# evfro/polara

Measured on AMD Instinct MI355X. Metric: users scored/sec + SVD build time, ML-20M rank-50 PureSVD, higher is better.
Workload: dtype bf16x3

## Files before the change

### include/polara_hip.h

```cpp
#ifndef POLARA_HIP_H
#define POLARA_HIP_H

#include <stdint.h>

#ifdef __cplusplus
extern "C" {
#endif

#define PK_OK 0
#define PK_E_INVALID (-1)
#define PK_E_LAUNCH (-2)
#define PK_E_UNSUPPORTED (-3)
#define PK_E_NOCONV (-4)

#define PK_VAL_F32 0
#define PK_VAL_F64 1

const char *pk_last_error(void);
int pk_version(void);
int pk_set_option(const char *name, int32_t value, int32_t unset);
int pk_copy_to_host_async(void *stream, void *dst_host, const void *src_dev, int64_t bytes);
int pk_device_info(int device, char *name, int name_len, int *cu_count, int64_t *hbm_bytes);
int pk_warm_up(void);

// ... 73 lines not shown
int pk_orth_check_f64(void *stream, int32_t l, const double *G_dev, int64_t ldg, int32_t *info_dev, int32_t n_info,
                      double *flags_dev);
int pk_eigh_psd_f64(void *stream, int32_t n, double *S_dev, int64_t lds_, double *evecs_dev, int64_t ldv,
                    double *evals_dev, int32_t max_sweeps, double tol, int32_t *info_dev);
int pk_eigh_psd_rounds_f64(void *stream, int32_t n, double *S_dev, int64_t lds_, double *evecs_dev, int64_t ldv,
                           double *evals_dev, int32_t max_sweeps, double tol, int32_t *info_dev);
int pk_eigh_top_supported(int32_t n, int32_t r);
int64_t pk_eigh_top_work_bytes(int32_t n);
int pk_eigh_top_f64(void *stream, int32_t n, const double *S_dev, int64_t lds_, int32_t r, double *evecs_dev, int64_t ldv,
                    double *evals_dev, void *work_dev, int32_t *info_dev);
int64_t pk_chol_work_bytes(int32_t n);
int pk_chol_rinv_f64(void *stream, int32_t n, const double *G_dev, int64_t ldg, double shift_rel, double *Rinv_dev,
                     int64_t ldr, void *work_dev, int32_t *info_dev);
int pk_chol_rinv_scaled_f64(void *stream, int32_t n, const double *G_dev, int64_t ldg, double shift_rel, double *Rinv_dev,
                     int64_t ldr, void *work_dev, int32_t *info_dev);
int pk_axpbypcz_f64(void *stream, int64_t n_elems, double alpha, const double *Z_dev, double beta,
                    const double *Y_dev, double gamma, const double *X_dev, double *out_dev);
int32_t pk_resid_blocks(int64_t n);
int pk_resid_colnorm2_f64(void *stream, int64_t n, int32_t l, const double *Z_dev, int64_t ldz,
                          const double *X_dev, int64_t ldx, const double *theta_dev, double *partial_dev);
int pk_dgemm_small_f64(void *stream, int transA, int transB, int32_t M, int32_t N, int32_t K,
                       const double *A_dev, int64_t lda, const double *B_dev, int64_t ldb,
                       double *C_dev, int64_t ldc);
int pk_scale_cols_f64(void *stream, int64_t n, int32_t l, double *X_dev, int64_t ldx, const double *s_dev);

int64_t pk_pack_elems(int64_t n, int32_t K);
int32_t pk_pack_kq(int32_t K);
int pk_pack_frag_f32(void *stream, int64_t n, int32_t K, const double *src_dev, int64_t ld, float *dst_dev);
int32_t pk_candidate_capacity(int32_t topk);
int64_t pk_score_state_bytes(int64_t n_users, int32_t splits);
int32_t pk_score_splits(int64_t n_users, int32_t KC);
int pk_seen_tiles_build(void *stream, int64_t n_users, const int64_t *seen_ptr_dev, const int32_t *seen_idx_dev,
                        int32_t rows_sorted ,
                        int64_t max_row_len ,
                        uint64_t *tiles_dev, int32_t *ntiles_dev);
int32_t pk_seen_tiles_max_unsorted_row(void);
int pk_score_candidates_f32(void *stream, int64_t n_users, int64_t n_items, int32_t K,
                            const float *Vp_dev, const float *Ep_dev,
                            const int64_t *seen_ptr_dev, const uint64_t *seen_tiles_dev,
                            const int32_t *seen_ntiles_dev ,
                            int32_t KC, int32_t splits ,
                            float *cand_score_dev, int32_t *cand_idx_dev ,
                            void *state_dev ,
                            int32_t tiles_per_chunk ,
                            const float *user_bound_dev ,
                            const float *tile_bound_dev ,
                            const uint32_t *seen_dense_dev, const int32_t *seen_skip_dev,
                            int32_t dense_tiles );
int pk_sweep_takes_rows(void);
int pk_score_candidates_rows_f32(void *stream, int64_t n_users, int64_t n_items, int32_t K, const float *Vp_dev,
                                 const double *E_dev, int64_t lde, const double *extra_dev, int64_t extra_ld,
                                 double extra_scale, const int64_t *seen_ptr_dev, const uint64_t *seen_tiles_dev,
                                 const int32_t *seen_ntiles_dev, int32_t KC, int32_t splits, float *cand_score_dev,
                                 int32_t *cand_idx_dev, void *state_dev, int32_t tiles_per_chunk ,
                                 const float *tile_bound_dev , const uint32_t *seen_dense_dev,
                                 const int32_t *seen_skip_dev, int32_t dense_tiles);
int pk_score_two_phase_plan(int64_t n_users, int64_t n_items, int32_t KC, int32_t *head_tiles, int32_t *splits);
int pk_score_two_phase_f32(void *stream, int64_t n_users, int64_t n_items, int32_t K,
                           const float *Vp_dev, const float *Ep_dev,
                           const int64_t *seen_ptr_dev, const uint64_t *seen_tiles_dev, const int32_t *seen_ntiles_dev,
                           int32_t KC, int32_t head_tiles, int32_t splits ,
                           float *work_score_dev, int32_t *work_idx_dev, float *cand_score_dev, int32_t *cand_idx_dev,
                           void *state_dev, int32_t tiles_per_chunk ,
                           const float *user_bound_dev, const float *tile_bound_dev ,
                           const uint32_t *seen_dense_dev, const int32_t *seen_skip_dev, int32_t dense_tiles);
int pk_score_two_phase_rows_f32(void *stream, int64_t n_users, int64_t n_items, int32_t K, const float *Vp_dev,
                                const double *E_dev, int64_t lde, const double *extra_dev, int64_t extra_ld,
                                double extra_scale, const int64_t *seen_ptr_dev, const uint64_t *seen_tiles_dev,
                                const int32_t *seen_ntiles_dev, int32_t KC, int32_t head_tiles, int32_t splits,
                                float *work_score_dev, int32_t *work_idx_dev, float *cand_score_dev, int32_t *cand_idx_dev,
                                void *state_dev, int32_t tiles_per_chunk, const float *tile_bound_dev,
                                const uint32_t *seen_dense_dev, const int32_t *seen_skip_dev, int32_t dense_tiles);
int64_t pk_seen_dense_bytes(int64_t n_users, int32_t dense_tiles);
int pk_seen_dense_build(void *stream, int64_t n_users, const int64_t *seen_ptr_dev, const uint64_t *seen_tiles_dev,
                        const int32_t *seen_ntiles_dev, int32_t dense_tiles, uint32_t *dense_dev, int32_t *skip_dev);
int32_t pk_score_chunk_launches(int64_t n_items, int32_t K, int32_t splits, int32_t tiles_per_chunk, int32_t pruned);
int pk_row_norm_bound_f32(void *stream, int64_t n, int32_t K, const double *src_dev, int64_t ld, float *out_dev);
int pk_v32_image_f32(void *stream, int64_t n, int32_t K, int32_t ld32, const double *V_dev, int64_t ldv, const float *bound_dev,
                     float *out_dev, uint32_t *stat_dev);
int pk_pack_frag_bound_f32(void *stream, int64_t n, int32_t K, const double *src_dev, int64_t ld, float *dst_dev,
                           float *bound_dev, const double *extra_dev, int64_t extra_ld, double extra_scale);
int pk_tile_norm_bound_f32(void *stream, int64_t n_items, int32_t K, const double *V_dev, int64_t ld,
                           float *work_dev, float *out_dev);
int pk_rescore_topk_f64(void *stream, int64_t n_users, int64_t n_items, int32_t K,
                        const double *V_dev, int64_t ldv, const double *E_dev, int64_t lde,
                        const int64_t *seen_ptr_dev, int32_t KC, int32_t splits,
                        const float *cand_score_dev, const int32_t *cand_idx_dev, int32_t topk,
                        double v_row_norm_max,
                        int64_t *out_idx_dev, double *out_score_dev , int32_t *flags_dev);
int pk_rescore_topk_rows_f64(void *stream, int64_t n_rows, const int32_t *rows_dev,
                             const int32_t *n_rows_dev ,
                             int64_t n_users, int64_t n_items,
                             int32_t K, const double *V_dev, int64_t ldv,
                             const float *V32_dev , int64_t ldv32,
                             const double *E_dev, int64_t lde,
                             const double *e_err_dev, int64_t e_err_ld ,
                             int32_t e_exact ,
                             const int64_t *seen_ptr_dev, int32_t KC, int32_t splits,
                             const float *cand_score_dev, const int32_t *cand_idx_dev, int32_t topk,
                             double v_row_norm_max,
                             int64_t *out_idx_dev, double *out_score_dev , int32_t *flags_dev);
int pk_rescore_topk_rows_list_f64(void *stream, int64_t n_rows, const int32_t *rows_dev,
                             const int32_t *n_rows_dev ,
                             int64_t n_users, int64_t n_items,
                             int32_t K, const double *V_dev, int64_t ldv,
                             const float *V32_dev , int64_t ldv32,
                             const double *E_dev, int64_t lde,
                             const double *e_err_dev, int64_t e_err_ld ,
                             int32_t e_exact ,
                             const int64_t *seen_ptr_dev, int32_t KC, int32_t splits,
                             const float *cand_score_dev, const int32_t *cand_idx_dev, int32_t topk,
                             double v_row_norm_max,
                             int64_t *out_idx_dev, double *out_score_dev , int32_t *flags_dev,
                             int32_t *flagged_list_dev, int32_t *flagged_count_dev, int32_t flagged_offset);
int pk_rescore_topk_rows_norms_f64(void *stream, int64_t n_rows, const int32_t *rows_dev,
                             const int32_t *n_rows_dev, int64_t n_users, int64_t n_items,
                             int32_t K, const double *V_dev, int64_t ldv,
                             const float *V32_dev, int64_t ldv32,
                             const double *E_dev, int64_t lde,
                             const double *e_err_dev, int64_t e_err_ld, int32_t e_exact,
                             const int64_t *seen_ptr_dev, int32_t KC, int32_t splits,
                             const float *cand_score_dev, const int32_t *cand_idx_dev, int32_t topk,
                             double v_row_norm_max,
                             int64_t *out_idx_dev, double *out_score_dev, int32_t *flags_dev,
                             int32_t *flagged_list_dev, int32_t *flagged_count_dev, int32_t flagged_offset,
                             const float *item_norm_dev);
int pk_rescore_topk_rows_perm_f64(void *stream, int64_t n_rows, const int32_t *rows_dev,
                             const int32_t *n_rows_dev, int64_t n_users, int64_t n_items,
                             int32_t K, const double *V_dev, int64_t ldv,
                             const float *V32_dev, int64_t ldv32,
                             const double *E_dev, int64_t lde,
                             const double *e_err_dev, int64_t e_err_ld, int32_t e_exact,
                             const int64_t *seen_ptr_dev, int32_t KC, int32_t splits,
                             const float *cand_score_dev, const int32_t *cand_idx_dev, int32_t topk,
                             double v_row_norm_max,
                             int64_t *out_idx_dev, double *out_score_dev, int32_t *flags_dev,
                             int32_t *flagged_list_dev, int32_t *flagged_count_dev, int32_t flagged_offset,
                             const float *item_norm_dev, const int64_t *out_perm_dev);
int pk_zero_i32(void *stream, int32_t *p_dev, int32_t n);
int pk_flag_compact(void *stream, int64_t n, const int32_t *flags_dev, int32_t mask, int32_t *list_dev,
                    int32_t *count_dev);
int pk_fold_rows_f64(void *stream, int64_t cap, const int32_t *list_dev, const int32_t *count_dev, int64_t row_offset,
                     const int64_t *indptr_dev, const int32_t *indices_dev, const void *vals_dev, int val_kind,
                     const double *V_dev, int64_t ldv, int32_t K, double *E_dev, int64_t lde);

int pk_spmm_csr_flagged_f64(void *stream, int64_t n_tasks, const int32_t *task_row_dev, const int64_t *task_begin_dev,
                            const int64_t *task_end_dev, const int32_t *task_slot_dev, int64_t n_long,
                            const int32_t *long_row_dev, const int32_t *long_slot_begin_dev,
                            const int32_t *long_slot_end_dev, const int32_t *indices_dev, const void *vals_dev,
                            int val_kind, const double *X_dev, int64_t ldx, int32_t nc, double *out_dev, int64_t ldo,
                            double *partial_dev, int64_t x_rows, const int32_t *row_flags_dev, int32_t flag_mask);

int pk_spmm_csr_rows_list_f64(void *stream, int64_t cap, const int32_t *list_dev, const int32_t *count_dev, int64_t row_offset,
                              const int64_t *row_first_task_dev, const int32_t *task_row_dev, const int64_t *task_begin_dev,
                              const int64_t *task_end_dev, const int32_t *task_slot_dev, int64_t n_long,
                              const int32_t *long_row_dev, const int32_t *long_slot_begin_dev, const int32_t *long_slot_end_dev,
                              const int32_t *indices_dev, const void *vals_dev, int val_kind, const double *X_dev, int64_t ldx,
                              int32_t nc, double *out_dev, int64_t ldo, double *partial_dev, int64_t x_rows,
                              const int32_t *row_flags_dev, int32_t flag_mask);

int32_t pk_q20_lanes(int32_t K);
double pk_q20_kappa(int32_t K);
int64_t pk_q20_image_bytes(int64_t n, int32_t K);
int pk_q20_encode_f64(void *stream, int64_t n, int32_t K, const double *V_dev, int64_t ldv, void *img_dev,
                      double *tab_dev, void *work_dev, int32_t *info_dev);
int pk_q20_decode_f64(void *stream, int64_t n, int32_t K, const void *img_dev, const double *tab_dev, double *out_dev,
// ... 167 lines not shown
```

### polara_amd/_lib.py

```python
import ctypes as C
import os

_HERE = os.path.dirname(os.path.abspath(__file__))
LIB_PATH = os.environ.get('POLARA_HIP_LIB') or os.path.join(_HERE, 'libpolarahip.so')

PK_VAL_F32, PK_VAL_F64 = 0, 1

_vp, _i32, _i64, _f64 = C.c_void_p, C.c_int32, C.c_int64, C.c_double

PROTOTYPES = {
    'pk_last_error': (C.c_char_p, []),
    'pk_version': (C.c_int, []),
    'pk_warm_up': (C.c_int, []),
    'pk_device_info': (C.c_int, [C.c_int, C.c_char_p, C.c_int, C.POINTER(C.c_int), C.POINTER(_i64)]),
    'pk_spmm_csr_f64': (C.c_int, [_vp, _i64, _vp, _vp, _vp, _vp, _i64, _vp, _vp, _vp, _vp, _vp, C.c_int,
                                  _vp, _i64, _i32, _vp, _i64, _vp]),
    'pk_spmm_csr_x': (C.c_int, [_vp, _i64, _vp, _vp, _vp, _vp, _i64, _vp, _vp, _vp, _vp, _vp, C.c_int,
                                _vp, C.c_int, _i64, _i32, _vp, _i64, _vp]),
    'pk_spmm_csr_ex': (C.c_int, [_vp, _i64, _vp, _vp, _vp, _vp, _i64, _vp, _vp, _vp, _vp, _vp, C.c_int,
                                 _vp, C.c_int, _i64, _i32, _vp, _i64, _vp, _i64, _i32, _i64]),
    'pk_scan_work_bytes': (_i64, [_i64]),
    'pk_exclusive_scan_i32': (C.c_int, [_vp, _i64, _vp, _vp, _vp]),
    'pk_radix_work_bytes': (_i64, [_i64]),
    'pk_radix_sort_pairs': (C.c_int, [_vp, _i64, _i32, _vp, _vp, _vp, _vp, _i32, _vp, C.POINTER(_i32)]),
    'pk_coo_to_csr_work_bytes': (_i64, [_i64]),
    'pk_coo_to_csr': (C.c_int, [_vp, _i64, _vp, _vp, _i64, _vp, C.c_int, _i64, _i64, _vp, _vp, _vp, _vp, _vp, _vp]),
    'pk_csr_transpose_work_bytes': (_i64, [_i64]),
    'pk_csr_transpose': (C.c_int, [_vp, _i64, _i64, _i64, _vp, _vp, _vp, C.c_int, _i64, _vp, _vp, _vp, _vp]),
    'pk_csr_relabel_work_bytes': (_i64, [_i64]),
    'pk_csr_relabel_sorted': (C.c_int, [_vp, _i64, _i64, _i64, _vp, _vp, _vp, C.c_int, _vp, _vp, _vp, _vp]),
    'pk_csr_rows_by_length_work_bytes': (_i64, [_i64]),
    'pk_csr_rows_by_length': (C.c_int, [_vp, _i64, _i64, _vp, _vp, _vp, C.c_int, _vp, _vp, _vp, _vp, _vp]),
    'pk_count_i32': (C.c_int, [_vp, _i64, _vp, _i64, _vp]),
    'pk_csr_scale_f64': (C.c_int, [_vp, _i64, _vp, _vp, _vp, C.c_int, _vp, _vp, _vp]),
    'pk_row_plan_work_bytes': (_i64, [_i64]),
    'pk_row_plan_count': (C.c_int, [_vp, _i64, _vp, _i32, _vp, _vp]),
    'pk_row_plan_fill': (C.c_int, [_vp, _i64, _vp, _vp, _vp, _vp, _vp, _vp, _vp, _vp, _vp, _vp, _vp]),
    'pk_gram_work_bytes': (_i64, [_i64, _i32, _i32]),
    'pk_gram_f64': (C.c_int, [_vp, _i64, _i32, _i32, _vp, _i64, _vp, _i64, _vp, _i64, _vp]),
    'pk_tsmm_f64': (C.c_int, [_vp, _i64, _i32, _i32, _vp, _i64, _vp, _i64, _vp, _i64]),
    'pk_tsmm_sub_f64': (C.c_int, [_vp, _i64, _i32, _i32, _vp, _i64, _vp, _i64, _vp, _i64, _vp, _i64]),
    'pk_tsmm_axpby_f64': (C.c_int, [_vp, _i64, _i32, _i32, _vp, _i64, _vp, _i64, _f64, _f64, _vp, _i64, _f64, _vp, _i64, _vp, _i64]),
    'pk_orth_check_f64': (C.c_int, [_vp, _i32, _vp, _i64, _vp, _i32, _vp]),
    'pk_eigh_psd_f64': (C.c_int, [_vp, _i32, _vp, _i64, _vp, _i64, _vp, _i32, _f64, _vp]),
    'pk_eigh_psd_rounds_f64': (C.c_int, [_vp, _i32, _vp, _i64, _vp, _i64, _vp, _i32, _f64, _vp]),
    'pk_eigh_top_supported': (C.c_int, [_i32, _i32]),
    'pk_eigh_top_work_bytes': (_i64, [_i32]),
    'pk_eigh_top_f64': (C.c_int, [_vp, _i32, _vp, _i64, _i32, _vp, _i64, _vp, _vp, _vp]),
    'pk_chol_work_bytes': (_i64, [_i32]),
    'pk_chol_rinv_f64': (C.c_int, [_vp, _i32, _vp, _i64, _f64, _vp, _i64, _vp, _vp]),
    'pk_chol_rinv_scaled_f64': (C.c_int, [_vp, _i32, _vp, _i64, _f64, _vp, _i64, _vp, _vp]),
    'pk_axpbypcz_f64': (C.c_int, [_vp, _i64, _f64, _vp, _f64, _vp, _f64, _vp, _vp]),
    'pk_resid_blocks': (_i32, [_i64]),
    'pk_resid_colnorm2_f64': (C.c_int, [_vp, _i64, _i32, _vp, _i64, _vp, _i64, _vp, _vp]),
    'pk_dgemm_small_f64': (C.c_int, [_vp, C.c_int, C.c_int, _i32, _i32, _i32, _vp, _i64, _vp, _i64, _vp, _i64]),
    'pk_scale_cols_f64': (C.c_int, [_vp, _i64, _i32, _vp, _i64, _vp]),
    'pk_pack_elems': (_i64, [_i64, _i32]),
    'pk_pack_kq': (_i32, [_i32]),
    'pk_pack_frag_f32': (C.c_int, [_vp, _i64, _i32, _vp, _i64, _vp]),
    'pk_candidate_capacity': (_i32, [_i32]),
    'pk_score_state_bytes': (_i64, [_i64, _i32]),
    'pk_score_splits': (_i32, [_i64, _i32]),
    'pk_seen_tiles_build': (C.c_int, [_vp, _i64, _vp, _vp, _i32, _i64, _vp, _vp]),
    'pk_seen_tiles_max_unsorted_row': (_i32, []),
    'pk_score_candidates_f32': (C.c_int, [_vp, _i64, _i64, _i32, _vp, _vp, _vp, _vp, _vp, _i32, _i32, _vp, _vp, _vp,
                                          _i32, _vp, _vp, _vp, _vp, _i32]),
    'pk_score_candidates_rows_f32': (C.c_int, [_vp, _i64, _i64, _i32, _vp, _vp, _i64, _vp, _i64, _f64, _vp, _vp, _vp, _i32, _i32,
                                               _vp, _vp, _vp, _i32, _vp, _vp, _vp, _i32]),
    'pk_score_two_phase_rows_f32': (C.c_int, [_vp, _i64, _i64, _i32, _vp, _vp, _i64, _vp, _i64, _f64, _vp, _vp, _vp, _i32, _i32, _i32,
                                              _vp, _vp, _vp, _vp, _vp, _i32, _vp, _vp, _vp, _i32]),
    'pk_score_two_phase_plan': (C.c_int, [_i64, _i64, _i32, _vp, _vp]),
    'pk_score_two_phase_f32': (C.c_int, [_vp, _i64, _i64, _i32, _vp, _vp, _vp, _vp, _vp, _i32, _i32, _i32, _vp, _vp, _vp, _vp, _vp,
                                         _i32, _vp, _vp, _vp, _vp, _i32]),
    'pk_seen_dense_bytes': (_i64, [_i64, _i32]),
    'pk_seen_dense_build': (C.c_int, [_vp, _i64, _vp, _vp, _vp, _i32, _vp, _vp]),
    'pk_score_chunk_launches': (_i32, [_i64, _i32, _i32, _i32, _i32]),
    'pk_pack_frag_bound_f32': (C.c_int, [_vp, _i64, _i32, _vp, _i64, _vp, _vp, _vp, _i64, _f64]),
    'pk_row_norm_bound_f32': (C.c_int, [_vp, _i64, _i32, _vp, _i64, _vp]),
    'pk_tile_norm_bound_f32': (C.c_int, [_vp, _i64, _i32, _vp, _i64, _vp, _vp]),
    'pk_rescore_topk_f64': (C.c_int, [_vp, _i64, _i64, _i32, _vp, _i64, _vp, _i64, _vp, _i32, _i32, _vp, _vp,
                                      _i32, _f64, _vp, _vp, _vp]),
    'pk_flag_compact': (C.c_int, [_vp, _i64, _vp, _i32, _vp, _vp]),
    'pk_fold_rows_f64': (C.c_int, [_vp, _i64, _vp, _vp, _i64, _vp, _vp, _vp, C.c_int, _vp, _i64, _i32, _vp, _i64]),
    'pk_spmm_csr_flagged_f64': (C.c_int, [_vp, _i64, _vp, _vp, _vp, _vp, _i64, _vp, _vp, _vp, _vp, _vp, C.c_int, _vp, _i64, _i32,
                                          _vp, _i64, _vp, _i64, _vp, _i32]),
    'pk_spmm_csr_rows_list_f64': (C.c_int, [_vp, _i64, _vp, _vp, _i64, _vp, _vp, _vp, _vp, _vp, _i64, _vp, _vp, _vp, _vp, _vp, C.c_int,
                                            _vp, _i64, _i32, _vp, _i64, _vp, _i64, _vp, _i32]),
    'pk_q20_lanes': (_i32, [_i32]),
    'pk_q20_kappa': (_f64, [_i32]),
    'pk_q20_image_bytes': (_i64, [_i64, _i32]),
    'pk_q20_encode_f64': (C.c_int, [_vp, _i64, _i32, _vp, _i64, _vp, _vp, _vp, _vp]),
    'pk_q20_decode_f64': (C.c_int, [_vp, _i64, _i32, _vp, _vp, _vp, _i64]),
    'pk_fold_q20': (C.c_int, [_vp, _i64, _vp, _vp, _vp, _vp, _i64, _vp, _vp, _vp, _vp, _vp, C.c_int, _vp, _vp, _i64, _i32, _i32,
                              _vp, _i64, _vp]),
    'pk_fold_q20_zero': (C.c_int, [_vp, _i64, _vp, _vp, _vp, _vp, _i64, _vp, _vp, _vp, _vp, _vp, C.c_int, _vp, _vp, _i64, _i32, _i32,
                                   _vp, _i64, _vp, _vp, _i32]),
    'pk_rescore_topk_rows_f64': (C.c_int, [_vp, _i64, _vp, _vp, _i64, _i64, _i32, _vp, _i64, _vp, _i64, _vp, _i64, _vp, _i64, _i32, _vp, _i32, _i32,
                                           _vp, _vp, _i32, _f64, _vp, _vp, _vp]),
    'pk_rescore_topk_rows_list_f64': (C.c_int, [_vp, _i64, _vp, _vp, _i64, _i64, _i32, _vp, _i64, _vp, _i64, _vp, _i64, _vp, _i64, _i32, _vp, _i32, _i32,
                                           _vp, _vp, _i32, _f64, _vp, _vp, _vp, _vp, _vp, _i32]),
    'pk_rescore_topk_rows_norms_f64': (C.c_int, [_vp, _i64, _vp, _vp, _i64, _i64, _i32, _vp, _i64, _vp, _i64, _vp, _i64, _vp, _i64, _i32, _vp, _i32, _i32,
                                           _vp, _vp, _i32, _f64, _vp, _vp, _vp, _vp, _vp, _i32, _vp]),
    'pk_rescore_topk_rows_perm_f64': (C.c_int, [_vp, _i64, _vp, _vp, _i64, _i64, _i32, _vp, _i64, _vp, _i64, _vp, _i64, _vp, _i64, _i32, _vp, _i32, _i32,
                                           _vp, _vp, _i32, _f64, _vp, _vp, _vp, _vp, _vp, _i32, _vp, _vp]),
    'pk_zero_i32': (C.c_int, [_vp, _vp, _i32]),
    'pk_scatter_rows_i64': (C.c_int, [_vp, _i64, _i32, _vp, _vp, _vp]),
    'pk_map_ids_i64': (C.c_int, [_vp, _i64, _vp, _vp, _i64, _vp]),
    'pk_exact_work_bytes': (_i64, [_i32, _i64]),
    'pk_score_exact_rows_f64': (C.c_int, [_vp, _i32, _vp, _i64, _i32, _vp, _i64, _vp, _i64, _vp, _vp, _i32,
                                          _vp, _vp, _vp]),
    'pk_score_exact_list_f64': (C.c_int, [_vp, _i32, _vp, _vp, _i64, _i32, _vp, _i64, _vp, _i64, _vp, _vp, _i32,
                                          _vp, _vp, _vp]),
    'pk_score_exact_list_perm_f64': (C.c_int, [_vp, _i32, _vp, _vp, _i64, _i32, _vp, _i64, _vp, _i64, _vp, _vp, _i32,
                                               _vp, _vp, _vp, _vp]),
    'pk_exact_work_init': (C.c_int, [_vp, _vp, _i32, _i64]),
    'pk_eval_ranks': (C.c_int, [_vp, _i64, _vp, _i32, _vp, _vp, _vp]),
    'pk_eval_cols': (_i32, []),
    'pk_eval_user_metrics': (C.c_int, [_vp, _i64, _i32, _vp, _i64, _vp, _vp, _vp, _vp, _f64, _f64, _i32, _vp]),
    'pk_eval_reduce_work_bytes': (_i64, [_i64]),
    'pk_eval_reduce': (C.c_int, [_vp, _i64, _vp, _vp, _vp]),
    'pk_unique_count_i64': (C.c_int, [_vp, _i64, _vp, _i64, _vp, _vp]),
    'pk_dense_scores_f64': (C.c_int, [_vp, _i32, _i64, _i32, _vp, _i64, _vp, _i64, _vp, _i64]),
    'pk_topk_rows_f64': (C.c_int, [_vp, _i64, _i64, _vp, _i64, _i32, _vp]),
    'pk_i2i_max_topk': (_i32, []),
    'pk_i2i_window': (_i32, []),
    'pk_i2i_build_window': (_i32, []),
    'pk_i2i_ld': (_i64, [_i64]),
    'pk_i2i_chunk_users': (_i64, [_i64, _i64, _i32]),
    'pk_i2i_topk_work_bytes': (_i64, [_i64, _i64, _i32]),
    'pk_i2i_build_f64': (C.c_int, [_vp, _i64, _i64, _vp, _vp, _vp, C.c_int, _vp, _vp, _vp, _vp, _i64]),
    'pk_i2i_image_f32': (C.c_int, [_vp, _i64, _vp, _vp, _vp]),
    'pk_i2i_topk': (C.c_int, [_vp, _i64, _i64, _vp, _vp, _vp, C.c_int, _vp, C.c_int, _i64, _i32, _i32, _i32, _vp, _vp, _vp]),
    'pk_popular_order_work_bytes': (_i64, [_i64]),
    'pk_popular_order': (C.c_int, [_vp, _i64, _vp, _vp, _vp]),
    'pk_popular_topk': (C.c_int, [_vp, _i64, _i64, _vp, _vp, _vp, _i32, _i32, _vp]),
    'pk_hybrid_ld': (_i64, [_i64]),
    'pk_hybrid_max_nc': (_i32, []),
    'pk_trmm_work_bytes': (_i64, [_i64, _i32]),
    'pk_hybrid_densify_f64': (C.c_int, [_vp, _i64, _vp, _vp, _vp, _vp, _f64, _vp, _i64]),
    'pk_chol_f64': (C.c_int, [_vp, _i64, _vp, _i64, _vp]),
    'pk_trmm_f64': (C.c_int, [_vp, _i32, _i64, _i32, _vp, _i64, _vp, _i64, _vp, _i64, _vp]),
    'pk_trsm_f64': (C.c_int, [_vp, _i64, _i32, _vp, _i64, _vp, _i64]),
    'pk_lce_fused_max_rank': (_i32, []),
    'pk_lce_update_f64': (C.c_int, [_vp, _i64, _i32, _vp, _i64, _vp, _i64, _vp, _i64, _f64, _vp, _i64, _f64, _f64, _f64, _vp]),
    'pk_lce_update_ew_f64': (C.c_int, [_vp, _i64, _i32, _vp, _i64, _vp, _i64, _vp, _i64, _f64, _f64, _vp]),
    'pk_lce_dot_blocks': (_i32, [_i64]),
    'pk_lce_dots_work_bytes': (_i64, []),
    'pk_lce_dots_f64': (C.c_int, [_vp, _i32, _vp, _vp, _vp, _vp, _vp, _vp, _vp, _vp, _f64, _vp, _vp]),
    'pk_clamp_min_f64': (C.c_int, [_vp, _i64, _i32, _vp, _i64, _f64]),
    'pk_ctx_create': (C.c_int, [_i32, C.POINTER(_vp)]),
    'pk_ctx_destroy': (None, [_vp]),
    'pk_ctx_error': (C.c_char_p, [_vp]),
    'pk_mat_from_csr': (C.c_int, [_vp, _i64, _i64, _i64, _vp, _vp, _vp, _i32, C.POINTER(_vp)]),
# ... 75 lines not shown
```

### polara_amd/csrc/api.cpp

```cpp
#include "pk_common.h"
#include <string.h>

static thread_local char g_err[512] = "";

void pk_set_error(const char *fmt, ...) {
    va_list ap;
    va_start(ap, fmt);
    vsnprintf(g_err, sizeof(g_err), fmt, ap);
    va_end(ap);
}

extern "C" const char *pk_last_error(void) { return g_err; }

#include <atomic>
namespace {
struct Option { const char *name; std::atomic<int> value; std::atomic<bool> set; };
Option g_options[] = {{"score_boot_tiles", {0}, {false}}, {"score_head_tiles", {0}, {false}}, {"score_phase2_splits", {0}, {false}}};
}
int pk_option(const char *name, int dflt) {
    for (auto &o : g_options)
        if (!strcmp(o.name, name)) return o.set.load() ? o.value.load() : dflt;
    return dflt;
}
extern "C" int pk_set_option(const char *name, int32_t value, int32_t unset) {
    if (name)
        for (auto &o : g_options)
            if (!strcmp(o.name, name)) {
                o.value.store(value);
                o.set.store(!unset);
                return PK_OK;
            }
    pk_set_error("pk_set_option: unknown option '%s'", name ? name : "(null)");
    return PK_E_INVALID;
}
extern "C" int pk_version(void) { return 100; }

extern "C" int pk_copy_to_host_async(void *stream, void *dst_host, const void *src_dev, int64_t bytes) {
    if (bytes < 0 || (bytes > 0 && (!dst_host || !src_dev))) {
        pk_set_error("pk_copy_to_host_async: bad arguments");
        return PK_E_INVALID;
    }
    if (bytes == 0) return PK_OK;
    const hipError_t e = hipMemcpyAsync(dst_host, src_dev, (size_t)bytes, hipMemcpyDeviceToHost, static_cast<hipStream_t>(stream));
    if (e != hipSuccess) {
        pk_set_error("pk_copy_to_host_async: %s", hipGetErrorString(e));
        return PK_E_LAUNCH;
    }
    return PK_OK;
}

extern "C" int pk_device_info(int device, char *name, int name_len, int *cu_count, int64_t *hbm_bytes) {
    int n = 0;
    hipError_t e = hipGetDeviceCount(&n);
    if (e != hipSuccess || n <= 0) {
        pk_set_error("pk_device_info: no HIP device visible (%s)", hipGetErrorString(e));
        return PK_E_LAUNCH;
    }
    if (device < 0 || device >= n) {
        pk_set_error("pk_device_info: device %d out of range [0,%d)", device, n);
        return PK_E_INVALID;
    }
    hipDeviceProp_t prop;
    e = hipGetDeviceProperties(&prop, device);
    if (e != hipSuccess) {
        pk_set_error("pk_device_info: %s", hipGetErrorString(e));
        return PK_E_LAUNCH;
    }
    if (name && name_len > 0) {
        strncpy(name, prop.gcnArchName, name_len - 1);
        name[name_len - 1] = 0;
    }
    if (cu_count) *cu_count = prop.multiProcessorCount;
    if (hbm_bytes) *hbm_bytes = (int64_t)prop.totalGlobalMem;
    return n;
}

hipError_t pk_tu_load_dense();
hipError_t pk_tu_load_driver();
hipError_t pk_tu_load_eigh();
hipError_t pk_tu_load_eigh_top();
hipError_t pk_tu_load_evalmetrics();
hipError_t pk_tu_load_hybrid();
hipError_t pk_tu_load_i2i();
hipError_t pk_tu_load_foldq();
hipError_t pk_tu_load_ingest();
hipError_t pk_tu_load_lce();
hipError_t pk_tu_load_rescore();
hipError_t pk_tu_load_score();
hipError_t pk_tu_load_spmm();
hipError_t pk_tu_load_ttm();

extern "C" int pk_warm_up(void) {
    hipError_t (*const loaders[])() = {pk_tu_load_dense, pk_tu_load_driver, pk_tu_load_eigh, pk_tu_load_eigh_top, pk_tu_load_evalmetrics, pk_tu_load_foldq, pk_tu_load_hybrid, pk_tu_load_i2i, pk_tu_load_ingest, pk_tu_load_lce, pk_tu_load_rescore, pk_tu_load_score, pk_tu_load_spmm, pk_tu_load_ttm};
    for (auto f : loaders) {
        const hipError_t e = f();
        if (e != hipSuccess) {
            pk_set_error("pk_warm_up: %s", hipGetErrorString(e));
            return PK_E_LAUNCH;
        }
    }
// ... 3 lines not shown
```

### polara_amd/csrc/driver.hip

```cpp
#include "pk_common.h"
#include <algorithm>
#include <cmath>
#include <cstdarg>
#include <cstring>
#include <map>
#include <memory>
#include <mutex>
#include <numeric>
#include <random>
#include <string>
#include <type_traits>
#include <vector>

namespace model {
constexpr double kDenseF64Flops = 20e12;
constexpr double kLanczosStepFixedS = 0.3e-3;
constexpr double kNestedSolveS = 1.5e-3;
constexpr double kXgmiBusBps = 100e9;
constexpr double kCollectiveStepS = 5e-6;
}

struct DevPool {
    std::multimap<size_t, void *> free_blocks;
    void *get(size_t &bytes) {
// ... 1682 lines not shown
    HIPCK(hipMemcpy2DAsync(Z_dev, (size_t)ldz * 8, Z.p(), (size_t)nc * 8, (size_t)nc * 8, (size_t)n, hipMemcpyDeviceToDevice, ctx->stream));
    return PK_OK;
}

__global__ void v32_image_stat_kernel(int64_t n, int K, int ld32, const double *__restrict__ V, int64_t ldv, const float *__restrict__ bound,
                                      float *__restrict__ out, uint32_t *__restrict__ stat) {
    const int64_t i = (int64_t)blockIdx.x * blockDim.x + threadIdx.x;
    if (i >= n * ld32) return;
    const int64_t r = i / ld32;
    const int c = (int)(i - r * ld32);
    float v = 0.0f;
    if (c < K) {
        const double d = V[r * ldv + c];
        v = (float)d;
        if (!(fabs(d) <= 1.7976931348623157e308)) atomicOr(&stat[1], 1u);
    } else if (c == K) {
        v = bound[r];
        if (!(v >= 0.0f && v <= 3.4028234e38f)) atomicOr(&stat[1], 1u); else atomicMax(&stat[0], __float_as_uint(v));
    }
    out[i] = v;
}

extern "C" int pk_v32_image_f32(void *stream, int64_t n, int32_t K, int32_t ld32, const double *V_dev, int64_t ldv, const float *bound_dev,
                                float *out_dev, uint32_t *stat_dev) {
    PK_REQUIRE(n >= 0 && K >= 1 && ld32 > K && ldv >= K && V_dev && bound_dev && out_dev && stat_dev, "pk_v32_image_f32: bad arguments");
    hipStream_t st = pk_stream(stream);
    (void)hipMemsetAsync(stat_dev, 0, 8, st);
    if (n > 0)
        hipLaunchKernelGGL(v32_image_stat_kernel, dim3((unsigned)(((size_t)n * ld32 + 255) / 256)), dim3(256), 0, st, n, K, ld32, V_dev, ldv, bound_dev,
                           out_dev, stat_dev);
    PK_CHECK_LAUNCH("v32_image_stat_kernel");
    return PK_OK;
}

extern "C" int pk_sym_eig_topk_f64(pk_ctx *ctx, void *stream, int32_t n, const double *T_dev, int64_t ldt, int32_t k, int32_t l,
                                   const double *X0_dev, int64_t ldx0, int32_t x0_rows, double tol, int32_t max_outer, uint64_t seed,
                                   double *basis_out_dev, int64_t ldb, double *lam_out_host, double *res_out_host,
                                   int32_t *counts_out, const double *lam0_host, double r0_rel) {
    if (!ctx) return PK_E_INVALID;
    std::lock_guard<std::mutex> lock(ctx->mu);
    PoolScope pool_scope(ctx);
    (void)hipSetDevice(ctx->device);
    if (n < 1 || k < 1 || l < k || l > n || l > 1024 || !T_dev || ldt < n || !basis_out_dev || ldb < l || !lam_out_host || !res_out_host ||
        !counts_out || (X0_dev && (x0_rows < 1 || x0_rows > n || ldx0 < l)))
        return fail(ctx, PK_E_INVALID, "pk_sym_eig_topk_f64: bad arguments (n=%d, k=%d, l=%d)", n, k, l);
    if (tol <= 0) tol = 1e-13;
    if (max_outer <= 0) max_outer = 200;
    hipStream_t st = stream ? pk_stream(stream) : ctx->stream;
    Solver S{ctx, st, Dev()};
    DMat T(n, n), X(n, l);
    if (!T.ok() || !X.ok()) return fail(ctx, PK_E_LAUNCH, "out of device memory (pk_sym_eig_topk_f64)");
    HIPCK(hipMemcpy2DAsync(T.p(), (size_t)n * 8, T_dev, (size_t)ldt * 8, (size_t)n * 8, (size_t)n, hipMemcpyDeviceToDevice, st));
    if (X0_dev) {
        HIPCK(hipMemsetAsync(X.p(), 0, (size_t)n * l * 8, st));
        HIPCK(hipMemcpy2DAsync(X.p(), (size_t)l * 8, X0_dev, (size_t)ldx0 * 8, (size_t)l * 8, (size_t)x0_rows, hipMemcpyDeviceToDevice, st));
    } else {
        hipLaunchKernelGGL(unit_block_kernel, dim3((unsigned)(((int64_t)n * l + 255) / 256)), dim3(256), 0, st, (int64_t)n, l, X.p());
    }
    DenseOp dop{ctx, S, T};
    SubspaceOut so;
    CK(dense_topk(ctx, S, dop, k, std::move(X), tol, max_outer, seed, X0_dev ? lam0_host : nullptr, r0_rel, so, X0_dev == nullptr));
    const int w = std::min<int>(l, so.basis.l);
    HIPCK(hipMemcpy2DAsync(basis_out_dev, (size_t)ldb * 8, so.basis.p(), (size_t)so.basis.l * 8, (size_t)w * 8, (size_t)n,
                           hipMemcpyDeviceToDevice, st));
    HIPCK(hipStreamSynchronize(st));
    for (int j = 0; j < l; ++j) lam_out_host[j] = j < (int)so.lam_all.size() ? so.lam_all[(size_t)j] : 0.0;
    for (int j = 0; j < l; ++j) res_out_host[j] = j < (int)so.res_act.size() ? so.res_act[(size_t)j] : 0.0;
    counts_out[0] = so.n_lock;
    counts_out[1] = w - so.n_lock;
    counts_out[2] = so.converged ? 1 : 0;
    counts_out[3] = so.outer;
    counts_out[4] = dop.products;
    return PK_OK;
}

struct pk_serving {
    int64_t n_items = 0, n_users = 0;
    int K = 0, ld32 = 0, Kx_full = 0;
    double vmax = 0.0;
    bool nonneg = true, have_tiles = false, have_v32 = false, fused = false;
    Dev inv64;
    DMat V;
    Csr Ts;
    Dev Vp, tile_bound, V32, tiles, ntiles, dense, skip;
    Dev vnorm, q20_raw, q20_tab;
    char *q20_img = nullptr;
    int dense_tiles = 0;
    Dev exact_work;
};

namespace {

int serving_build(pk_ctx *ctx, pk_serving *sv, int64_t n_items, int32_t K, const double *V_host, pk_mat *T) {
    hipStream_t st = ctx->stream;
    const int64_t n_users = T->A.n_rows;
    Solver S{ctx, st, Dev()};
    sv->n_items = n_items; sv->n_users = n_users; sv->K = K; sv->nonneg = T->nonneg; sv->fused = K <= 256;
    std::vector<double> norm((size_t)n_items, 0.0);
    for (int j = 0; j < K; ++j)
        for (int64_t i = 0; i < n_items; ++i) { const double v = V_host[(size_t)j * n_items + i]; norm[(size_t)i] += v * v; }
    double vmax = 0.0;
    for (auto &v : norm) { v = std::sqrt(v); vmax = std::max(vmax, v); }
    if (!std::isfinite(vmax) || (vmax != 0.0 && !(vmax > 1e-30 && vmax < 1e30)))
        return fail(ctx, PK_E_INVALID, "pk_score_topk: item factors with max row norm %g are outside the fp32 range of the candidate sweep", vmax);
    sv->vmax = vmax;
    std::vector<int32_t> inv((size_t)n_items), rank_of((size_t)n_items);
    std::iota(inv.begin(), inv.end(), 0);
    std::stable_sort(inv.begin(), inv.end(), [&](int32_t a, int32_t b) { return norm[(size_t)a] > norm[(size_t)b]; });
    for (int64_t i = 0; i < n_items; ++i) rank_of[(size_t)inv[(size_t)i]] = (int32_t)i;
    {
        std::vector<int64_t> inv_l(inv.begin(), inv.end());
        if (!sv->inv64.alloc((size_t)n_items * 8)) return fail(ctx, PK_E_LAUNCH, "out of device memory (item ids)");
        CK(S.upload(inv_l.data(), sv->inv64.p, (size_t)n_items * 8));
    }
    std::vector<double> vr((size_t)n_items * K);
    for (int64_t i = 0; i < n_items; ++i)
        for (int j = 0; j < K; ++j) vr[(size_t)i * K + j] = V_host[(size_t)j * n_items + inv[(size_t)i]];
    sv->V = DMat(n_items, K);
    DMat &V = sv->V;
    if (!V.ok()) return fail(ctx, PK_E_LAUNCH, "out of device memory (factors)");
    CK(S.upload(vr.data(), V.p(), vr.size() * 8));
    Csr &Ts = sv->Ts;
    Ts.n_rows = n_users; Ts.n_cols = n_items; Ts.nnz = T->A.nnz; Ts.val_kind = T->A.val_kind;
    const size_t ve = Ts.val_kind == PK_VAL_F32 ? 4 : 8, n1 = (size_t)std::max<int64_t>(Ts.nnz, 1);
    {
        Dev cmap((size_t)n_items * 4), work((size_t)pk_csr_relabel_work_bytes(Ts.nnz));
        if (!cmap.p || !work.p || !Ts.indptr.alloc((size_t)(n_users + 1) * 8) || !Ts.indices.alloc(n1 * 4) || !Ts.values.alloc(n1 * ve))
            return fail(ctx, PK_E_LAUNCH, "out of device memory (test matrix)");
        CK(S.upload(rank_of.data(), cmap.p, (size_t)n_items * 4));
        HIPCK(hipMemcpyAsync(Ts.indptr.p, T->A.indptr.p, (size_t)(n_users + 1) * 8, hipMemcpyDeviceToDevice, st));
        CK(pk_csr_relabel_sorted(st, n_users, n_items, Ts.nnz, T->A.indptr.as<int64_t>(), T->A.indices.as<int32_t>(), T->A.values.p,
                                 Ts.val_kind, cmap.as<int32_t>(), Ts.indices.as<int32_t>(), Ts.values.p, work.p));
        HIPCK(hipStreamSynchronize(st));
    }
    CK(build_plan(ctx, Ts));
    if (!sv->fused) return PK_OK;
    Dev tb_work((size_t)n_items * 4), rowb((size_t)n_items * 4);
    if (!sv->Vp.alloc((size_t)pk_pack_elems(n_items, K) * 4) || !sv->tile_bound.alloc((size_t)((n_items + 31) / 32) * 4) || !tb_work.p || !rowb.p)
        return fail(ctx, PK_E_LAUNCH, "out of device memory (factor images)");
    CK(pk_pack_frag_f32(st, n_items, K, V.p(), K, sv->Vp.as<float>()));
    CK(pk_tile_norm_bound_f32(st, n_items, K, V.p(), K, tb_work.as<float>(), sv->tile_bound.as<float>()));
    sv->Kx_full = ((K + 1 + 3) / 4) * 4;
    sv->ld32 = sv->Kx_full > 16 ? ((sv->Kx_full + 31) / 32) * 32 : (sv->Kx_full <= 4 ? 4 : sv->Kx_full <= 8 ? 8 : 16);
    if (sv->Kx_full <= 256 && sv->nonneg) {
        if (!sv->V32.alloc((size_t)n_items * sv->ld32 * 4)) return fail(ctx, PK_E_LAUNCH, "out of device memory (fp32 image)");
        CK(pk_row_norm_bound_f32(st, n_items, K, V.p(), K, rowb.as<float>()));
        hipLaunchKernelGGL(v32_image_kernel, dim3((unsigned)(((size_t)n_items * sv->ld32 + 255) / 256)), dim3(256), 0, st, n_items, K, sv->ld32,
                           V.p(), rowb.as<float>(), sv->V32.as<float>());
        sv->have_v32 = true;
        if (!sv->vnorm.alloc((size_t)n_items * 4)) return fail(ctx, PK_E_LAUNCH, "out of device memory (item norms)");
        HIPCK(hipMemcpyAsync(sv->vnorm.p, rowb.p, (size_t)n_items * 4, hipMemcpyDeviceToDevice, st));
        const int64_t qbytes = pk_q20_image_bytes(n_items, K);
        if (qbytes > 0 && n_items < (1 << 24) && qbytes < ((int64_t)1 << 32)) {
            Dev qwork(768), qinfo(4);
            if (!sv->q20_raw.alloc((size_t)qbytes + 128) || !sv->q20_tab.alloc(96 * 8) || !qwork.p || !qinfo.p)
                return fail(ctx, PK_E_LAUNCH, "out of device memory (packed image)");
            char *img = static_cast<char *>(sv->q20_raw.p);
            img += (128 - (reinterpret_cast<uintptr_t>(img) & 127)) & 127;
            CK(pk_q20_encode_f64(st, n_items, K, V.p(), K, img, sv->q20_tab.as<double>(), qwork.p, qinfo.as<int32_t>()));
            int32_t info = 0;
            CK(S.to_host(qinfo.p, &info, 4));
            if (info == 0) sv->q20_img = img;
        }
    }
    HIPCK(hipStreamSynchronize(st));
    return PK_OK;
}

int serving_score(pk_ctx *ctx, pk_serving *sv, int32_t topk, int32_t filter_seen, int64_t *out_idx, double *out_scores) {
    hipStream_t st = ctx->stream;
    const int64_t n_items = sv->n_items, n_users = sv->n_users;
    const int K = sv->K;
    if (!out_idx || topk < 1) return fail(ctx, PK_E_INVALID, "pk_score_topk: bad arguments");
    if (topk > n_items) return fail(ctx, PK_E_INVALID, "kth(=%lld) out of bounds (%lld)", (long long)(n_items - topk), (long long)n_items);
    Solver S{ctx, st, Dev()};
    DMat &V = sv->V;
    Csr &Ts = sv->Ts;
    const double vmax = sv->vmax;
    const size_t n1 = (size_t)std::max<int64_t>(Ts.nnz, 1);
    const Range all{0, Ts.plan.n_tasks, 0, Ts.plan.n_long};
    const int64_t *seen_ptr = filter_seen ? Ts.indptr.as<int64_t>() : nullptr;
    const int32_t *seen_idx = filter_seen ? Ts.indices.as<int32_t>() : nullptr;
    Dev out_i((size_t)n_users * topk * 8), out_s((size_t)n_users * topk * 8), flags((size_t)n_users * 4), lst((size_t)std::max<int64_t>(n_users, 1) * 4), cnt(4);
    Dev lst2((size_t)std::max<int64_t>(n_users, 1) * 4), cnt2(8);
    if (!out_i.p || !out_s.p || !flags.p || !lst.p || !cnt.p || !lst2.p || !cnt2.p) return fail(ctx, PK_E_LAUNCH, "out of device memory (outputs)");
    const int KC = sv->fused ? pk_candidate_capacity(topk) : 0;
    const int n_wg = 128;
    Dev &exact_work = sv->exact_work;
    if (!exact_work.p) {
        if (!exact_work.alloc((size_t)pk_exact_work_bytes(n_wg, n_items))) return fail(ctx, PK_E_LAUNCH, "out of device memory (exact rows)");
        CK(pk_exact_work_init(st, exact_work.p, n_wg, n_items));
    }
    if (KC == 0) {
        DMat E(n_users, K);
        if (!E.ok()) return fail(ctx, PK_E_LAUNCH, "out of device memory (E)");
        CK(spmm(ctx, Ts, V.p(), PK_VAL_F64, K, K, E.p(), K, all));
        hipLaunchKernelGGL(iota_i32_kernel, dim3((unsigned)((n_users + 255) / 256)), dim3(256), 0, st, n_users, lst.as<int32_t>(), cnt.as<int32_t>());
        CK(pk_score_exact_list_f64(st, n_wg, lst.as<int32_t>(), cnt.as<int32_t>(), n_items, K, V.p(), K, E.p(), K, seen_ptr, seen_idx, topk,
                                   out_i.as<int64_t>(), out_s.as<double>(), exact_work.p));
        HIPCK(hipStreamSynchronize(st));
    } else {
        const bool approx = !out_scores && sv->have_v32;
        const int Kx = approx ? sv->Kx_full : K, ld32 = sv->ld32;
        DMat Ex(n_users, Kx);
        if (!Ex.ok()) return fail(ctx, PK_E_LAUNCH, "out of device memory (E)");
        bool counters_zeroed = false;
        if (approx && sv->q20_img && topk <= 20) {
            Plan &P = Ts.plan;
            const size_t need = (size_t)P.n_slots * Kx * 8;
            if (need > P.partial.bytes && !P.partial.alloc(need)) return fail(ctx, PK_E_LAUNCH, "out of device memory (fold-in partials)");
            CK(pk_fold_q20_zero(st, all.nt, P.task_row.as<int32_t>() + all.t0, P.task_begin.as<int64_t>() + all.t0,
                                P.task_end.as<int64_t>() + all.t0, P.task_slot.as<int32_t>() + all.t0, all.nl,
                                P.long_row.as<int32_t>() + all.l0, P.long_sb.as<int32_t>() + all.l0, P.long_se.as<int32_t>() + all.l0,
                                Ts.indices.as<int32_t>(), Ts.values.p, Ts.val_kind, sv->q20_img, sv->q20_tab.as<double>(), n_items, K, Kx,
                                Ex.p(), Kx, P.partial.as<double>(), cnt2.as<int32_t>(), 2));
            counters_zeroed = true;
        } else if (approx) CK(spmm(ctx, Ts, sv->V32.p, PK_VAL_F32, ld32, Kx, Ex.p(), Kx, all));
        else CK(spmm(ctx, Ts, V.p(), PK_VAL_F64, K, K, Ex.p(), Kx, all));
        const double *w = approx ? Ex.p() + K : nullptr;
        const bool from_rows = (Kx % 2 == 0) && (((uintptr_t)Ex.p()) % 16 == 0);
        Dev Ep, ub;
        if (!from_rows) {
            if (!Ep.alloc((size_t)pk_pack_elems(n_users, K) * 4) || !ub.alloc((size_t)n_users * 4))
                return fail(ctx, PK_E_LAUNCH, "out of device memory (E fragments)");
            CK(pk_pack_frag_bound_f32(st, n_users, K, Ex.p(), Kx, Ep.as<float>(), ub.as<float>(), w, approx ? Kx : 0, 1.2e-7));
        }
        if (filter_seen && !sv->have_tiles) {
            if (!sv->tiles.alloc(n1 * 8) || !sv->ntiles.alloc((size_t)n_users * 4)) return fail(ctx, PK_E_LAUNCH, "out of device memory (seen tiles)");
            CK(pk_seen_tiles_build(st, n_users, Ts.indptr.as<int64_t>(), Ts.indices.as<int32_t>(), 1, 0, sv->tiles.as<uint64_t>(), sv->ntiles.as<int32_t>()));
            sv->have_tiles = true;
            const int64_t n_tiles_all = (n_items + 31) / 32, groups = (n_users + 31) / 32;
            int dt = (int)std::min<int64_t>(n_tiles_all, 256);
            while (dt > 32 && groups * dt * 128 > ((int64_t)512 << 20)) dt /= 2;
            if (n_tiles_all <= 32 * (int64_t)dt && sv->dense.alloc((size_t)pk_seen_dense_bytes(n_users, dt)) &&
                sv->skip.alloc((size_t)n_users * 4)) {
                CK(pk_seen_dense_build(st, n_users, Ts.indptr.as<int64_t>(), sv->tiles.as<uint64_t>(), sv->ntiles.as<int32_t>(), dt,
                                       sv->dense.as<uint32_t>(), sv->skip.as<int32_t>()));
                sv->dense_tiles = dt;
            }
        }
        const uint64_t *tiles = filter_seen ? sv->tiles.as<uint64_t>() : nullptr;
        const int32_t *ntiles = filter_seen ? sv->ntiles.as<int32_t>() : nullptr;
        int splits = ((n_users + 31) / 32) * 8 > 2048 ? 1 : pk_score_splits(n_users, KC);
        const int64_t n_pad = ((n_users + 31) / 32) * 32;
        int32_t head_tiles = 0, splits2 = 0;
        CK(pk_score_two_phase_plan(n_users, n_items, KC, &head_tiles, &splits2));
        const int slots = head_tiles ? splits2 + 1 : splits;
        Dev state((size_t)pk_score_state_bytes(n_users, slots)), cs((size_t)slots * n_pad * KC * 4), ci((size_t)slots * n_pad * KC * 4);
        Dev ms(head_tiles ? (size_t)n_pad * KC * 4 : 0), mi(head_tiles ? (size_t)n_pad * KC * 4 : 0);
        if (!state.p || !cs.p || !ci.p || (head_tiles && (!ms.p || !mi.p))) return fail(ctx, PK_E_LAUNCH, "out of device memory (candidates)");
        const uint32_t *dense_p = (filter_seen && sv->dense_tiles) ? sv->dense.as<uint32_t>() : nullptr;
        const int32_t *skip_p = (filter_seen && sv->dense_tiles) ? sv->skip.as<int32_t>() : nullptr;
        if (head_tiles) {
            if (from_rows)
                CK(pk_score_two_phase_rows_f32(st, n_users, n_items, K, sv->Vp.as<float>(), Ex.p(), Kx, w, approx ? Kx : 0, 1.2e-7, seen_ptr,
                                               tiles, ntiles, KC, head_tiles, splits2, cs.as<float>(), ci.as<int32_t>(), ms.as<float>(),
                                               mi.as<int32_t>(), state.p, 0, sv->tile_bound.as<float>(), dense_p, skip_p,
                                               filter_seen ? sv->dense_tiles : 0));
            else
                CK(pk_score_two_phase_f32(st, n_users, n_items, K, sv->Vp.as<float>(), Ep.as<float>(), seen_ptr, tiles, ntiles, KC, head_tiles,
                                          splits2, cs.as<float>(), ci.as<int32_t>(), ms.as<float>(), mi.as<int32_t>(), state.p, 0, ub.as<float>(),
                                          sv->tile_bound.as<float>(), dense_p, skip_p, filter_seen ? sv->dense_tiles : 0));
            std::swap(cs, ms);
            std::swap(ci, mi);
            splits = 1;
        } else if (from_rows) {
            CK(pk_score_candidates_rows_f32(st, n_users, n_items, K, sv->Vp.as<float>(), Ex.p(), Kx, w, approx ? Kx : 0, 1.2e-7, seen_ptr,
                                            tiles, ntiles, KC, splits, cs.as<float>(), ci.as<int32_t>(), state.p, 0,
                                            sv->tile_bound.as<float>(), dense_p, skip_p, filter_seen ? sv->dense_tiles : 0));
        } else {
            CK(pk_score_candidates_f32(st, n_users, n_items, K, sv->Vp.as<float>(), Ep.as<float>(), seen_ptr, tiles, ntiles,
                                       KC, splits, cs.as<float>(), ci.as<int32_t>(), state.p, 0, ub.as<float>(), sv->tile_bound.as<float>(),
                                       dense_p, skip_p, filter_seen ? sv->dense_tiles : 0));
        }
        if (!counters_zeroed) CK(pk_zero_i32(st, cnt2.as<int32_t>(), 2));
        int32_t *c_refold = cnt2.as<int32_t>(), *c_final = cnt2.as<int32_t>() + 1;
        CK(pk_rescore_topk_rows_norms_f64(st, n_users, nullptr, nullptr, n_users, n_items, K, V.p(), K, approx ? sv->V32.as<float>() : nullptr, approx ? ld32 : 0,
                                          Ex.p(), Kx, w, approx ? Kx : 0, 0, seen_ptr, KC, splits, cs.as<float>(), ci.as<int32_t>(), topk, vmax,
                                          out_i.as<int64_t>(), out_s.as<double>(), flags.as<int32_t>(),
                                          approx ? lst.as<int32_t>() : lst2.as<int32_t>(), approx ? c_refold : c_final, 0,
                                          approx ? sv->vnorm.as<float>() : nullptr));
        if (approx) {
            if ((K & 1) == 0 && K >= 2) {
                Plan &P = Ts.plan;
                const size_t need = (size_t)P.n_slots * K * 8;
                if (need > P.partial.bytes && !P.partial.alloc(need)) return fail(ctx, PK_E_LAUNCH, "out of device memory (re-fold partials)");
                CK(pk_spmm_csr_rows_list_f64(st, n_users, lst.as<int32_t>(), c_refold, 0, P.row_first_task.as<int64_t>(), P.task_row.as<int32_t>(),
                                             P.task_begin.as<int64_t>(), P.task_end.as<int64_t>(), P.task_slot.as<int32_t>(), all.nl,
                                             P.long_row.as<int32_t>() + all.l0, P.long_sb.as<int32_t>() + all.l0, P.long_se.as<int32_t>() + all.l0,
                                             Ts.indices.as<int32_t>(), Ts.values.p, Ts.val_kind, V.p(), K, K, Ex.p(), Kx, P.partial.as<double>(),
                                             n_items, flags.as<int32_t>(), 7));
            } else
            CK(pk_fold_rows_f64(st, n_users, lst.as<int32_t>(), c_refold, 0, Ts.indptr.as<int64_t>(), Ts.indices.as<int32_t>(), Ts.values.p,
                                Ts.val_kind, V.p(), K, K, Ex.p(), Kx));
            CK(pk_rescore_topk_rows_list_f64(st, n_users, lst.as<int32_t>(), c_refold, n_users, n_items, K, V.p(), K, nullptr, 0, Ex.p(), Kx, w, Kx,
                                             1, seen_ptr, KC, splits, cs.as<float>(), ci.as<int32_t>(), topk, vmax, out_i.as<int64_t>(), out_s.as<double>(),
                                             flags.as<int32_t>(), lst2.as<int32_t>(), c_final, 0));
        }
        CK(pk_score_exact_list_f64(st, n_wg, lst2.as<int32_t>(), c_final, n_items, K, V.p(), K, Ex.p(), Kx, seen_ptr, seen_idx, topk,
                                   out_i.as<int64_t>(), out_s.as<double>(), exact_work.p));
        HIPCK(hipStreamSynchronize(st));
    }
    Dev ext((size_t)n_users * topk * 8);
    if (!ext.p) return fail(ctx, PK_E_LAUNCH, "out of device memory (outputs)");
    CK(pk_map_ids_i64(st, n_users * (int64_t)topk, out_i.as<int64_t>(), sv->inv64.as<int64_t>(), n_items, ext.as<int64_t>()));
    CK(S.to_host(ext.p, out_idx, (size_t)n_users * topk * 8));
    if (out_scores) CK(S.to_host(out_s.p, out_scores, (size_t)n_users * topk * 8));
    return PK_OK;
}

}

extern "C" int pk_serving_create(pk_ctx *ctx, int64_t n_items, int32_t K, const double *V_host, pk_mat *T, pk_serving **out) {
    if (!ctx || !T || !out) return PK_E_INVALID;
    std::lock_guard<std::mutex> lock(ctx->mu);
    PoolScope pool_scope(ctx);
    (void)hipSetDevice(ctx->device);
    *out = nullptr;
    if (n_items != T->A.n_cols) return fail(ctx, PK_E_INVALID, "pk_score_topk: test matrix and item factors disagree on the number of items");
    if (K < 1 || K > 8192 || !V_host) return fail(ctx, PK_E_INVALID, "pk_score_topk: bad arguments");
    std::unique_ptr<pk_serving> sv(new pk_serving());
    const int rc = serving_build(ctx, sv.get(), n_items, K, V_host, T);
    if (rc != PK_OK) return rc;
    *out = sv.release();
    return PK_OK;
}

extern "C" int pk_serving_score(pk_ctx *ctx, pk_serving *sv, int32_t topk, int32_t filter_seen, int64_t *out_idx, double *out_scores) {
    if (!ctx || !sv) return PK_E_INVALID;
    std::lock_guard<std::mutex> lock(ctx->mu);
    PoolScope pool_scope(ctx);
    (void)hipSetDevice(ctx->device);
    return serving_score(ctx, sv, topk, filter_seen, out_idx, out_scores);
}

extern "C" void pk_serving_free(pk_ctx *ctx, pk_serving *sv) {
    if (!sv) return;
    if (ctx) {
        std::lock_guard<std::mutex> lock(ctx->mu);
        PoolScope pool_scope(ctx);
        (void)hipStreamSynchronize(ctx->stream);
        delete sv;
    } else {
        delete sv;
    }
}

extern "C" int pk_score_topk(pk_ctx *ctx, int64_t n_items, int32_t K, const double *V_host, pk_mat *T, int32_t topk,
                             int32_t filter_seen, int64_t *out_idx, double *out_scores) {
    if (!ctx || !T) return PK_E_INVALID;
    std::lock_guard<std::mutex> lock(ctx->mu);
    PoolScope pool_scope(ctx);
// ... 295 lines not shown
```

### polara_amd/csrc/score.hip

```cpp
#include "pk_common.h"
#include <math.h>
#include <stdlib.h>

typedef float f32x16 __attribute__((ext_vector_type(16)));
typedef __bf16 bf16x8 __attribute__((ext_vector_type(8)));

#define RING 16

#define PK_IDX_NONE 0x7fffffff
#define PK_IDX_FLOOR (-2)
#define PK_TILE_NONE 0xffffffff00000000ull

template <int K, int J, int S>
constexpr unsigned long long pk_wave_stage_mask() {
    unsigned long long m = 0;
    for (int l = 0; l < 64; ++l) {
        const int i = l + 64 * S;
        if (((i & J) == 0) == ((i & K) == 0)) m |= 1ull << l;
    }
    return m;
}
template <int SLOTS, int K, int J>
__device__ __forceinline__ void pk_sort32_stage(unsigned (&key)[SLOTS]) {
    if constexpr (J >= 64) {
// ... 12 lines not shown
            const unsigned hi = key[1] > other[1] ? key[1] : other[1], lo = key[1] > other[1] ? other[1] : key[1];
            key[1] = __builtin_amdgcn_inverse_ballot_w64(pk_wave_stage_mask<K, J, 1>()) ? hi : lo;
        }
    }
}
template <int SLOTS, int K, int J>
__device__ __forceinline__ void pk_sort32_merge(unsigned (&key)[SLOTS]) {
    pk_sort32_stage<SLOTS, K, J>(key);
    if constexpr (J > 1) pk_sort32_merge<SLOTS, K, (J >> 1)>(key);
}
template <int SLOTS, int K>
__device__ __forceinline__ void pk_sort32_levels(unsigned (&key)[SLOTS]) {
    if constexpr (K > 2) pk_sort32_levels<SLOTS, (K >> 1)>(key);
    pk_sort32_merge<SLOTS, K, (K >> 1)>(key);
}
template <int SLOTS>
__device__ __forceinline__ void pk_sort32_wave_desc(unsigned (&key)[SLOTS]) {
    static_assert(SLOTS == 1 || SLOTS == 2, "pk_sort32_wave_desc: 64 or 128 elements");
    pk_sort32_levels<SLOTS, 64 * SLOTS>(key);
}

template <int K, int J>
constexpr unsigned long long pk_half_stage_mask() {
    unsigned long long m = 0;
    for (int l = 0; l < 64; ++l) {
        const int t = l & 31;
        if (((t & J) == 0) == ((t & K) == 0)) m |= 1ull << l;
    }
    return m;
}
template <int K, int J>
__device__ __forceinline__ void pk_sort32_half_merge(unsigned &key) {
    const unsigned other = (unsigned)pk_lane_xor<J>((int)key);
    const unsigned hi = key > other ? key : other, lo = key > other ? other : key;
    key = __builtin_amdgcn_inverse_ballot_w64(pk_half_stage_mask<K, J>()) ? hi : lo;
    if constexpr (J > 1) pk_sort32_half_merge<K, (J >> 1)>(key);
}
template <int K>
__device__ __forceinline__ void pk_sort32_half_levels(unsigned &key) {
    if constexpr (K > 2) pk_sort32_half_levels<(K >> 1)>(key);
    pk_sort32_half_merge<K, (K >> 1)>(key);
}
__device__ __forceinline__ unsigned pk_float_order(float x) {
    const unsigned u = __float_as_uint(x);
    return (u & 0x80000000u) ? ~u : (u | 0x80000000u);
}

__device__ __forceinline__ unsigned pk_bf16_rne(float x) {
    unsigned u = __float_as_uint(x);
    u += 0x7fffu + ((u >> 16) & 1u);
    return u >> 16;
}
__device__ __forceinline__ void pk_split_bf16(float x, unsigned &hi, unsigned &lo) {
    hi = pk_bf16_rne(x);
    lo = pk_bf16_rne(x - __uint_as_float(hi << 16));
}

struct LaneState {
    int64_t sp;
    float tau;
    int cnt;
};
#define PK_LANE_DONE (-1)

__host__ __device__ constexpr bool pk_top_in_lds(int nstep, int kc) { return kc <= 32 || nstep > 8; }
__host__ __device__ constexpr int pk_ring_rows(int nstep, int kc) { return kc == 16 ? 8 : ((nstep > 8 && kc == 64) ? 2 * RING : RING); }
__host__ __device__ constexpr size_t pk_score_lds_bytes(int nstep, int kc) {
    return (size_t)(4 * pk_ring_rows(nstep, kc) * 64 + (pk_top_in_lds(nstep, kc) ? 4 * 32 * kc : 1)) * sizeof(uint2);
}
struct SeenDense {
    const unsigned *mask;
    const int32_t *skip;
    int tiles;
};

struct UserRows {
    const double *E;
    int64_t ld;
    int K;
    const double *extra;
    int64_t extra_ld;
    double extra_scale;
};

template <int NSTEP, int KC, bool STRIDED, bool DENSE>
__global__ __launch_bounds__(256) void score_candidates_kernel(
    const float4 *__restrict__ Vp, const float4 *__restrict__ Ep, int64_t n_users, int n_items,
    int n_tiles, int split_tiles, int chunk_begin, int chunk_tiles,
    const int64_t *__restrict__ seen_ptr, const unsigned long long *__restrict__ seen_tiles,
    const int32_t *__restrict__ seen_ntiles,
    float *__restrict__ cand_score, int32_t *__restrict__ cand_idx,
    LaneState *__restrict__ st_lane, uint2 *__restrict__ st_ring,
    const float *__restrict__ user_bound, const float *__restrict__ tile_bound, SeenDense dense,
    int tile_base, int slot_base, const LaneState *__restrict__ floor_state, int boot_tiles, UserRows rows) {
    constexpr int KQ = 2 * NSTEP;
    constexpr bool PAIRED = (KC == 16);
    constexpr int RG = pk_ring_rows(NSTEP, KC);
    constexpr int SLOTS = (2 * RG + KC + 63) / 64;
    constexpr bool TOP_LDS = pk_top_in_lds(NSTEP, KC);
    extern __shared__ __attribute__((aligned(16))) uint2 pk_score_lds[];
    constexpr int NW = 4;

    const int lane = threadIdx.x & 63;
    const int wave = __builtin_amdgcn_readfirstlane((int)(threadIdx.x >> 6));
    const int64_t group_raw = (int64_t)blockIdx.x * NW + wave;
    if (group_raw * 32 >= n_users) return;
    const int64_t group = group_raw;
    uint2(*ring)[64] = reinterpret_cast<uint2(*)[64]>(pk_score_lds + wave * (RG * 64));
    uint2 *top = pk_score_lds + NW * RG * 64 + (TOP_LDS ? wave * (32 * KC) : 0);

    const int split = STRIDED ? (int)blockIdx.y : 0;
    const int S = STRIDED ? (int)gridDim.y : 1;
    const int64_t n_groups = (n_users + 31) / 32;
    const int t_lo = tile_base + split;
    const int tile_begin = t_lo + chunk_begin * S;
    const int tile_stop = (chunk_begin + chunk_tiles < split_tiles) ? t_lo + (chunk_begin + chunk_tiles) * S : n_tiles;
    const int tile_end = (tile_stop < n_tiles) ? tile_stop : n_tiles;
    const bool first = (chunk_begin == 0);
    const bool last = (tile_stop >= n_tiles);
    if (!first && tile_begin >= n_tiles) return;

    const int ul = lane & 31, hi = lane >> 5;
    const int64_t user = group * 32 + ul;
    const int64_t slot = (int64_t)(slot_base + split) * n_groups + group;
    float *my_score = cand_score + slot * 32 * KC;
    int32_t *my_idx = cand_idx + slot * 32 * KC;

    float4 e[KQ];
    float en_rows = -1.0f;
    if (rows.E) {
        double *buf = reinterpret_cast<double *>(&ring[0][0]);
        double ss = 0.0;
#pragma unroll
        for (int s = 0; s < NSTEP; ++s) {
            __builtin_amdgcn_wave_barrier();
#pragma unroll
            for (int p = 0; p < 4; ++p) {
                const int rr = 8 * p + (lane >> 3);
                const int kk = 16 * s + 2 * (lane & 7);
                const int64_t grow = group * 32 + rr;
                double2 v = make_double2(0.0, 0.0);
                if (grow < n_users && kk < rows.K) {
                    const double *g = rows.E + grow * rows.ld + kk;
                    if (kk + 1 < rows.K) v = *reinterpret_cast<const double2 *>(g);
                    else v.x = g[0];
                }
                *reinterpret_cast<double2 *>(buf + rr * 16 + 2 * (lane & 7)) = v;
            }
            __builtin_amdgcn_wave_barrier();
            unsigned bh[8], bl[8];
            const double *mine = buf + ul * 16 + 8 * hi;
#pragma unroll
            for (int j = 0; j < 8; ++j) {
                const double x = mine[j];
                ss = fma(x, x, ss);
                pk_split_bf16((float)x, bh[j], bl[j]);
            }
            e[2 * s] = __builtin_bit_cast(float4, make_uint4(bh[0] | (bh[1] << 16), bh[2] | (bh[3] << 16), bh[4] | (bh[5] << 16), bh[6] | (bh[7] << 16)));
            e[2 * s + 1] = __builtin_bit_cast(float4, make_uint4(bl[0] | (bl[1] << 16), bl[2] | (bl[3] << 16), bl[4] | (bl[5] << 16), bl[6] | (bl[7] << 16)));
        }
        __builtin_amdgcn_wave_barrier();
        ss += pk_lane_xor<32>(ss);
        if (user < n_users) {
            double b = sqrt(ss) * (1.0 + 1e-6);
            if (rows.extra) b += rows.extra_scale * rows.extra[user * rows.extra_ld];
            en_rows = (float)(b * (1.0 + 1e-7));
        }
    } else {
#pragma unroll
        for (int q = 0; q < KQ; ++q) e[q] = Ep[(group * KQ + q) * 64 + lane];
    }

    int64_t sp = 0, se = 0;
    unsigned long long nxt = PK_TILE_NONE, nxt2 = PK_TILE_NONE, nxt3 = PK_TILE_NONE;
    float tau = -INFINITY;
    int cnt = 0;
    const bool prune = (user_bound != nullptr || rows.E != nullptr) && tile_bound != nullptr;
    const float en = (prune && user < n_users) ? (rows.E ? en_rows : user_bound[user]) : -1.0f;
    bool pruned = false;
    int exit_tile = tile_end;
    const bool has_seen = (seen_ptr != nullptr && user < n_users);
    if (has_seen) {
        sp = seen_ptr[user];
        se = sp + seen_ntiles[user];
    }
    LaneState *my_state = st_lane + slot * 64 + lane;
    uint2 *my_ring_state = st_ring + slot * (RING * 64);
    float tau_floor = -INFINITY;
    if constexpr (STRIDED) {
        if (floor_state) {
            const LaneState fs = floor_state[group * 64 + lane];
            if ((int)fs.sp < tile_base) {
                if (first) {
                    for (int s = lane; s < 32 * KC; s += 64) {
                        my_score[s] = -INFINITY;
                        my_idx[s] = -1;
                    }
                    LaneState ls;
                    ls.sp = fs.sp;
                    ls.tau = fs.tau;
                    ls.cnt = PK_LANE_DONE;
                    *my_state = ls;
                }
                return;
            }
            tau_floor = fs.tau;
            tau = tau_floor;
        }
    }
    const int dense_tiles = (DENSE && seen_ptr != nullptr) ? dense.tiles : 0;
    const unsigned *dense_row = dense_tiles ? dense.mask + ((int64_t)group * dense_tiles) * 32 + ul : nullptr;
    if (DENSE && first && has_seen && dense_tiles) sp += dense.skip[user];
    if (first) {
        if (has_seen && t_lo > 0 && !(DENSE && dense_tiles >= t_lo)) {
            int64_t lo = sp, hi_ = se;
            while (lo < hi_) {
                const int64_t mid = (lo + hi_) >> 1;
                if ((unsigned)(seen_tiles[mid] >> 32) < (unsigned)t_lo) lo = mid + 1; else hi_ = mid;
            }
            sp = lo;
        }
        for (int s = lane; s < 32 * KC; s += 64) {
            if (TOP_LDS) {
                top[s] = make_uint2(__float_as_uint(-INFINITY), 0xffffffffu);
            } else {
                my_score[s] = -INFINITY;
                my_idx[s] = -1;
            }
        }
    } else {
        const LaneState ls = *my_state;
        if (ls.cnt == PK_LANE_DONE) {
            return;
        }
        if (TOP_LDS)
            for (int s = lane; s < 32 * KC; s += 64) top[s] = make_uint2(__float_as_uint(my_score[s]), (unsigned)my_idx[s]);
        if (has_seen) sp = ls.sp;
        tau = ls.tau;
        tau_floor = fmaxf(tau_floor, tau);
        cnt = ls.cnt;
        const int cmax = __builtin_amdgcn_readfirstlane((int)__reduce_max_sync(~0ull, cnt));
        for (int i = 0; i < cmax; ++i) ring[i][lane] = my_ring_state[i * 64 + lane];
    }
    if (has_seen) {
        if (sp < se) nxt = seen_tiles[sp];
        if (sp + 1 < se) nxt2 = seen_tiles[sp + 1];
        if (sp + 2 < se) nxt3 = seen_tiles[sp + 2];
    }

// ... 288 lines not shown
                    c = acc[r] > tau;
                }
                if (c) {
                    ring[cnt][lane] = make_uint2(__float_as_uint(acc[r]),
                                                 (unsigned)(j0 + (r & 3) + 8 * (r >> 2) + 4 * hi));
                    ++cnt;
                }
            }
        }
    };
    auto score_tile_roll = [&](float4(&a)[KQ], int next_tile) -> f32x16 {
        f32x16 acc;
#pragma unroll
        for (int r = 0; r < 16; ++r) acc[r] = 0.0f;
        const float4 *vp = Vp + ((int64_t)next_tile * KQ) * 64 + lane;
#pragma unroll
        for (int sidx = 0; sidx < NSTEP; ++sidx) {
            const bf16x8 vh = __builtin_bit_cast(bf16x8, a[2 * sidx]), vl = __builtin_bit_cast(bf16x8, a[2 * sidx + 1]);
            const bf16x8 eh = __builtin_bit_cast(bf16x8, e[2 * sidx]), el = __builtin_bit_cast(bf16x8, e[2 * sidx + 1]);
            acc = __builtin_amdgcn_mfma_f32_32x32x16_bf16(vh, eh, acc, 0, 0, 0);
            acc = __builtin_amdgcn_mfma_f32_32x32x16_bf16(vh, el, acc, 0, 0, 0);
            acc = __builtin_amdgcn_mfma_f32_32x32x16_bf16(vl, eh, acc, 0, 0, 0);
            a[2 * sidx] = vp[(2 * sidx) * 64];
            a[2 * sidx + 1] = vp[(2 * sidx + 1) * 64];
        }
        return acc;
    };
    if (first && boot_tiles > 0 && floor_state == nullptr) {
        constexpr int BL = KC / 2;
        constexpr int BG = KC / 8;
        float bl[BL];
#pragma unroll
        for (int i = 0; i < BL; ++i) bl[i] = -INFINITY;
        const int64_t sp0 = sp;
        const unsigned long long n0 = nxt, n1 = nxt2, n2 = nxt3;
        float4 a_nxt[KQ];
        load_frags((tile_begin < n_tiles) ? tile_begin : 0, a_nxt);
        unsigned m_nxt = 0u;
        if constexpr (DENSE) m_nxt = (tile_begin < dense_tiles) ? dense_row[(int64_t)tile_begin * 32] : 0u;
        for (int i = 0, tile = tile_begin; i < boot_tiles && tile < tile_end; ++i, tile += S) {
            {
                if constexpr (DENSE) {
                    m_dense = m_nxt;
                    m_nxt = (tile + S < dense_tiles) ? dense_row[(int64_t)(tile + S) * 32] : 0u;
                }
                f32x16 acc;
                acc = score_tile_roll(a_nxt, (tile + S < tile_end) ? tile + S : tile);
                const unsigned m2 = walk_mask(tile) >> (4 * hi);
#pragma unroll
                for (int g = 0; g < BG; ++g) {
                    float x = -INFINITY;
#pragma unroll
                    for (int r = g * (16 / BG); r < (g + 1) * (16 / BG); ++r)
                        x = fmaxf(x, (m2 & (1u << ((r & 3) + 8 * (r >> 2)))) ? -INFINITY : acc[r]);
#pragma unroll
                    for (int i2 = 0; i2 < BL; ++i2) {
                        const float up = fmaxf(bl[i2], x);
                        x = fminf(bl[i2], x);
                        bl[i2] = up;
                    }
                }
            }
        }
        float t0 = bl[KC / 2 - 1];
        t0 = fminf(t0, __int_as_float(pk_lane_xor<32>(__float_as_int(t0))));
        if (t0 > -INFINITY) {
            t0 = fminf(t0 - fabsf(t0) * 2.4e-7f, t0 - 1e-37f);
            tau_floor = fmaxf(tau_floor, t0);
            tau = fmaxf(tau, tau_floor);
        }
        sp = sp0;
        nxt = n0;
        nxt2 = n1;
        nxt3 = n2;
        has_pend = false;
    }
    {
        {
        float4 a_nxt[KQ];
        load_frags((tile_begin < n_tiles) ? tile_begin : 0, a_nxt);
        unsigned m_nxt = 0u;
        if constexpr (DENSE) m_nxt = (tile_begin < dense_tiles) ? dense_row[(int64_t)tile_begin * 32] : 0u;
        float tb = prune ? tile_bound[(tile_begin < n_tiles) ? tile_begin : 0] : 0.0f;
        int step = 0;
        for (int tile = tile_begin; tile < tile_end; tile += S, ++step) {
            if (prune) {
                const bool open = en * tb > tau;
                const unsigned long long ob = __ballot(open);
                if (ob == 0ull) {
                    pruned = true;
                    exit_tile = tile;
                    break;
                } else {
                    if (((STRIDED ? step : tile) & 7) == 7 && __popcll(ob) <= 16) {
                        const unsigned long long pend = __ballot(cnt > 0);
                        flush_set((unsigned)(ob | (ob >> 32)) & (unsigned)(pend | (pend >> 32)));
                    }
                    tb = tile_bound[(tile + S < n_tiles) ? tile + S : tile];
                }
            }
            {
                if constexpr (DENSE) {
                    m_dense = m_nxt;
                    m_nxt = (tile + S < dense_tiles) ? dense_row[(int64_t)(tile + S) * 32] : 0u;
                }
                f32x16 acc;
                acc = score_tile_roll(a_nxt, (tile + S < tile_end) ? tile + S : tile);
                const unsigned mask = walk_mask(tile);
                float m_all = fmaxf(acc[0], acc[1]);
#pragma unroll
                for (int r = 2; r < 16; ++r) m_all = fmaxf(m_all, acc[r]);
                if (__any(m_all > tau)) {
                    float sc[16];
                    float m = m_all;
                    if (__any(mask != 0)) {
                        const unsigned m2 = mask >> (4 * hi);
#pragma unroll
                        for (int r = 0; r < 16; ++r)
                            sc[r] = (m2 & (1u << ((r & 3) + 8 * (r >> 2)))) ? -INFINITY : acc[r];
                        m = fmaxf(sc[0], sc[1]);
#pragma unroll
                        for (int r = 2; r < 16; ++r) m = fmaxf(m, sc[r]);
                    } else {
#pragma unroll
                        for (int r = 0; r < 16; ++r) sc[r] = acc[r];
                    }
                    if (__any(m > tau)) push_candidates(sc, tile * 32);
                }
            }
        }
        }
    }

    if (!last && !pruned) {
        if constexpr (RG > RING) {
            const unsigned long long over = __ballot(cnt > RING);
            flush_set((unsigned)(over | (over >> 32)));
        }
        LaneState ls;
        ls.sp = sp;
        ls.tau = tau;
        ls.cnt = cnt;
        *my_state = ls;
        const int cmax = __builtin_amdgcn_readfirstlane((int)__reduce_max_sync(~0ull, cnt));
        __builtin_amdgcn_wave_barrier();
        for (int i = 0; i < cmax; ++i) my_ring_state[i * 64 + lane] = ring[i][lane];
        if (TOP_LDS)
            for (int s = lane; s < 32 * KC; s += 64) {
                const uint2 r = top[s];
                my_score[s] = __uint_as_float(r.x);
                my_idx[s] = (int)r.y;
            }
        return;
    }
    {
        const unsigned long long some = __ballot(cnt > 0);
        flush_set((unsigned)(some | (some >> 32)));
    }
    const unsigned long long floored = (floor_state == nullptr) ? __ballot(tau_floor > -INFINITY) : 0ull;
    if (TOP_LDS) {
        __builtin_amdgcn_wave_barrier();
        for (int s = lane; s < 32 * KC; s += 64) {
            const uint2 r = top[s];
            int iv = (int)r.y;
            if ((s % KC) == KC - 1 && iv < 0 && ((floored >> (s / KC)) & 1ull)) iv = PK_IDX_FLOOR;
            my_score[s] = __uint_as_float(r.x);
            my_idx[s] = iv;
        }
    } else if (floored) {
        __builtin_amdgcn_fence(__ATOMIC_RELEASE, "workgroup");
// ... 262 lines not shown
    }
    hipLaunchKernelGGL(seen_dense_kernel, dim3((unsigned)pk_ceil_div(n_users, 4)), dim3(256), 0, st, n_users, seen_ptr_dev,
                       reinterpret_cast<const unsigned long long *>(seen_tiles_dev), seen_ntiles_dev, dense_tiles, dense_dev,
                       skip_dev);
    PK_CHECK_LAUNCH("seen_dense_kernel");
    return PK_OK;
}

extern "C" int pk_seen_tiles_build(void *stream, int64_t n_users, const int64_t *seen_ptr_dev,
                                   const int32_t *seen_idx_dev, int32_t rows_sorted, int64_t max_row_len,
                                   uint64_t *tiles_dev, int32_t *ntiles_dev) {
    PK_REQUIRE(n_users >= 1 && seen_ptr_dev && ntiles_dev, "pk_seen_tiles_build: bad arguments");
    dim3 grid((unsigned)pk_ceil_div(n_users, 4)), block(256);
    unsigned long long *tiles = reinterpret_cast<unsigned long long *>(tiles_dev);
    if (rows_sorted) {
        hipLaunchKernelGGL(seen_tiles_kernel<true>, grid, block, 0, pk_stream(stream), n_users, seen_ptr_dev,
                           seen_idx_dev, tiles, ntiles_dev);
    } else {
        PK_REQUIRE(max_row_len >= 0 && max_row_len <= PK_SEEN_CAP,
                   "pk_seen_tiles_build: unsorted rows longer than %d entries (got %lld): sort the rows first",
                   PK_SEEN_CAP, (long long)max_row_len);
        hipLaunchKernelGGL(seen_tiles_kernel<false>, grid, block, 0, pk_stream(stream), n_users, seen_ptr_dev,
                           seen_idx_dev, tiles, ntiles_dev);
    }
    PK_CHECK_LAUNCH("seen_tiles_kernel");
    return PK_OK;
}

__global__ __launch_bounds__(256) void row_norm_bound_kernel(int64_t n, int K, const double *__restrict__ src,
                                                             int64_t ld, float *__restrict__ out) {
    const int64_t r = ((int64_t)blockIdx.x * blockDim.x + threadIdx.x) >> 4;
    const int l = threadIdx.x & 15;
    double s = 0.0;
    if (r < n) {
        const double *row = src + r * ld;
        for (int k = l; k < K; k += 16) s = fma(row[k], row[k], s);
    }
#pragma unroll
    for (int off = 8; off > 0; off >>= 1) s += __shfl_xor(s, off, 64);
    if (r < n && l == 0) out[r] = (float)(sqrt(s) * (1.0 + 1e-6));
}

__global__ __launch_bounds__(64) void tile_suffix_max_kernel(int64_t n, int64_t n_tiles, const float *__restrict__ norm,
                                                             float *__restrict__ out) {
    const int lane = threadIdx.x;
    const int64_t seg = (n_tiles + 63) / 64;
    const int64_t t0 = lane * seg, t1 = (t0 + seg < n_tiles) ? t0 + seg : n_tiles;
    float run = 0.0f;
    for (int64_t t = t1 - 1; t >= t0; --t) {
        const int64_t i1 = (32 * t + 32 < n) ? 32 * t + 32 : n;
        for (int64_t i = 32 * t; i < i1; ++i) run = fmaxf(run, norm[i]);
        out[t] = run;
    }
    float carry = 0.0f;
    for (int l = 63; l > 0; --l) {
        const float v = __shfl(run, l);
        if (lane < l) carry = fmaxf(carry, v);
    }
    for (int64_t t = t0; t < t1; ++t) out[t] = fmaxf(out[t], carry);
}

extern "C" int pk_row_norm_bound_f32(void *stream, int64_t n, int32_t K, const double *src_dev, int64_t ld,
                                     float *out_dev) {
    PK_REQUIRE(n >= 1 && K >= 1 && ld >= K, "pk_row_norm_bound_f32: bad sizes");
    hipLaunchKernelGGL(row_norm_bound_kernel, dim3((unsigned)pk_ceil_div(n, 16)), dim3(256), 0, pk_stream(stream), n,
                       K, src_dev, ld, out_dev);
    PK_CHECK_LAUNCH("row_norm_bound_kernel");
    return PK_OK;
}

extern "C" int pk_tile_norm_bound_f32(void *stream, int64_t n_items, int32_t K, const double *V_dev, int64_t ld,
                                      float *work_dev, float *out_dev) {
    PK_REQUIRE(n_items >= 1 && K >= 1 && ld >= K, "pk_tile_norm_bound_f32: bad sizes");
    hipStream_t st = pk_stream(stream);
    hipLaunchKernelGGL(row_norm_bound_kernel, dim3((unsigned)pk_ceil_div(n_items, 16)), dim3(256), 0, st, n_items, K,
                       V_dev, ld, work_dev);
    PK_CHECK_LAUNCH("row_norm_bound_kernel");
    hipLaunchKernelGGL(tile_suffix_max_kernel, dim3(1), dim3(64), 0, st, n_items, pk_ceil_div(n_items, 32), work_dev,
                       out_dev);
    PK_CHECK_LAUNCH("tile_suffix_max_kernel");
    return PK_OK;
}

extern "C" int32_t pk_candidate_capacity(int32_t topk) {
    if (topk < 1) return 0;
    if (topk <= 10) return 16;
    if (topk <= 24) return 32;
    if (topk <= 52) return 64;
    return 0;
}

#define PK_CHUNK_BYTES (2560 * 1024)

struct SweepPhase {
    int tile_base;
    int slot_base;
    const LaneState *floor_state;
    int boot_tiles;
};

template <int NSTEP>
static int launch_candidates_n(hipStream_t st, int KC, dim3 grid, const float4 *Vp, const float4 *Ep,
                               int64_t n_users, int n_items, int n_tiles, int split_tiles, int tiles_per_chunk,
                               const int64_t *seen_ptr, const unsigned long long *seen_tiles,
                               const int32_t *seen_ntiles, float *cs, int32_t *ci,
                               LaneState *st_lane, uint2 *st_ring, const float *user_bound, const float *tile_bound,
                               SeenDense dense, SweepPhase ph, UserRows rows) {
    constexpr bool DENSE_OK = (NSTEP <= 8);
    const bool use_dense = dense.tiles > 0 && DENSE_OK && (grid.y == 1 || ph.floor_state != nullptr);
    const SeenDense no_dense{nullptr, nullptr, 0};
    const SeenDense dn = use_dense ? dense : no_dense;
    int chunk_tiles = tiles_per_chunk;
    for (int chunk_begin = 0; chunk_begin < split_tiles; chunk_begin += chunk_tiles, chunk_tiles = (tile_bound ? 2 * chunk_tiles : chunk_tiles)) {
#define PK_LAUNCH(KCV)                                                                                          \
    if (pk_score_lds_bytes(NSTEP, KCV) > 64 * 1024) {                                                           \
        static PkDeviceOnce attr_set;              \
        if (attr_set.pending()) {                                                                                        \
            hipError_t e1 = hipFuncSetAttribute(reinterpret_cast<const void *>(&score_candidates_kernel<NSTEP, KCV, false, false>), \
                                                hipFuncAttributeMaxDynamicSharedMemorySize,                     \
                                                (int)pk_score_lds_bytes(NSTEP, KCV));                           \
            if (e1 == hipSuccess)                                                                               \
                e1 = hipFuncSetAttribute(reinterpret_cast<const void *>(&score_candidates_kernel<NSTEP, KCV, true, DENSE_OK>), \
                                         hipFuncAttributeMaxDynamicSharedMemorySize,                            \
                                         (int)pk_score_lds_bytes(NSTEP, KCV));                                  \
            if (e1 != hipSuccess) {                                                                             \
                pk_set_error("pk_score_candidates_f32: cannot raise the LDS limit: %s", hipGetErrorString(e1)); \
                return PK_E_LAUNCH;                                                                             \
            }                                                                                                   \
            attr_set.done();                                                                                       \
        }                                                                                                       \
    }                                                                                                           \
    if (grid.y > 1 || ph.floor_state != nullptr)                                                                \
        hipLaunchKernelGGL((score_candidates_kernel<NSTEP, KCV, true, DENSE_OK>), grid, dim3(256), pk_score_lds_bytes(NSTEP, KCV), st, Vp, Ep, n_users, \
                           n_items, n_tiles, split_tiles, chunk_begin, chunk_tiles, seen_ptr, seen_tiles, seen_ntiles, cs, ci, st_lane, st_ring,  \
                           user_bound, tile_bound, dn, ph.tile_base, ph.slot_base, ph.floor_state, ph.boot_tiles, rows); \
    else if (use_dense)                                                                                         \
        hipLaunchKernelGGL((score_candidates_kernel<NSTEP, KCV, false, DENSE_OK>), grid, dim3(256), pk_score_lds_bytes(NSTEP, KCV), st, Vp, Ep, n_users, \
                           n_items, n_tiles, split_tiles, chunk_begin, chunk_tiles, seen_ptr, seen_tiles, seen_ntiles, cs, ci, st_lane, st_ring,  \
                           user_bound, tile_bound, dn, 0, ph.slot_base, nullptr, ph.boot_tiles, rows);  \
    else                                                                                                        \
        hipLaunchKernelGGL((score_candidates_kernel<NSTEP, KCV, false, false>), grid, dim3(256), pk_score_lds_bytes(NSTEP, KCV), st, Vp, Ep, n_users, \
                           n_items, n_tiles, split_tiles, chunk_begin, chunk_tiles, seen_ptr, seen_tiles, seen_ntiles, cs, ci, st_lane, st_ring,  \
                           user_bound, tile_bound, no_dense, 0, ph.slot_base, nullptr, ph.boot_tiles, rows)
        switch (KC) {
            case 16:
                PK_LAUNCH(16);
                break;
            case 32:
                PK_LAUNCH(32);
                break;
            case 64:
                PK_LAUNCH(64);
                break;
            default:
                pk_set_error("pk_score_candidates_f32: KC=%d unsupported (16, 32, 64)", KC);
                return PK_E_UNSUPPORTED;
        }
#undef PK_LAUNCH
    }
    return PK_OK;
}

extern "C" int64_t pk_score_state_bytes(int64_t n_users, int32_t splits) {
    const int64_t slots = pk_ceil_div(n_users, 32) * (splits < 1 ? 1 : splits);
    return slots * 64 * (int64_t)sizeof(LaneState) + slots * RING * 64 * (int64_t)sizeof(uint2);
}

extern "C" int32_t pk_score_splits(int64_t n_users, int32_t KC) {
    const int64_t groups = pk_ceil_div(n_users, 32);
    const int64_t slots = 256 * 8;
    int64_t s = (groups > 0) ? slots / groups : 1;
    const int smax = 64 / (KC > 0 ? KC : 64);
    if (s > smax) s = smax;
    if (s < 1) s = 1;
    return (int32_t)s;
}

static int pk_auto_chunk_tiles(int kq, int splits, int split_tiles, bool pruned) {
    if (pruned) return split_tiles > 8 ? split_tiles : 8;
    int t = PK_CHUNK_BYTES / (kq * 1024) / splits;
    return t < 8 ? 8 : t;
}

extern "C" int32_t pk_score_chunk_launches(int64_t n_items, int32_t K, int32_t splits, int32_t tiles_per_chunk,
                                           int32_t pruned) {
    const int kq = pk_pack_kq(K);
    if (kq <= 0 || n_items < 1 || splits < 1) return 0;
    const int n_tiles = (int)pk_ceil_div(n_items, 32);
    const int split_tiles = (int)pk_ceil_div(n_tiles, splits);
    if (tiles_per_chunk <= 0) tiles_per_chunk = pk_auto_chunk_tiles(kq, splits, split_tiles, pruned != 0);
    int n = 0, ct = tiles_per_chunk;
    for (int b = 0; b < split_tiles; b += ct, ct = (pruned ? 2 * ct : ct)) ++n;
    return n;
}

static int pk_sweep_launches(hipStream_t st, int64_t n_users, int64_t n_items, int n_tiles, int32_t K, const float *Vp_dev,
                             const float *Ep_dev, const int64_t *seen_ptr_dev, const uint64_t *seen_tiles_dev,
                             const int32_t *seen_ntiles_dev, int32_t KC, int32_t splits, int32_t total_slots,
                             float *cand_score_dev, int32_t *cand_idx_dev, void *state_dev, int32_t tiles_per_chunk,
                             const float *user_bound_dev, const float *tile_bound_dev, SeenDense dense, SweepPhase ph,
                             UserRows rows = UserRows{nullptr, 0, 0, nullptr, 0, 0.0}) {
    const int kq = pk_pack_kq(K);
    const int nstep = pk_nstep(K);
    const int64_t groups = pk_ceil_div(n_users, 32);
    const int split_tiles = (int)pk_ceil_div(n_tiles - ph.tile_base, splits);
    if (tiles_per_chunk <= 0) tiles_per_chunk = pk_auto_chunk_tiles(kq, splits, split_tiles, tile_bound_dev != nullptr);
    LaneState *st_lane = static_cast<LaneState *>(state_dev);
    uint2 *st_ring = reinterpret_cast<uint2 *>(st_lane + groups * total_slots * 64);
    if (ph.floor_state) ph.floor_state = st_lane;
    ph.boot_tiles = ph.floor_state ? 0 : pk_option("score_boot_tiles", 16);
    dim3 grid((unsigned)pk_ceil_div(groups, 4), (unsigned)splits);
    const float4 *Vp = reinterpret_cast<const float4 *>(Vp_dev);
    const float4 *Ep = reinterpret_cast<const float4 *>(Ep_dev);
    int rc = PK_E_UNSUPPORTED;
#define PK_N_CASE(Q)                                                                                          \
    case Q:                                                                                                   \
        rc = launch_candidates_n<Q>(st, KC, grid, Vp, Ep, n_users, (int)n_items, n_tiles,            \
                                    split_tiles, tiles_per_chunk, seen_ptr_dev,                                   \
                                    reinterpret_cast<const unsigned long long *>(seen_tiles_dev), seen_ntiles_dev, \
                                    cand_score_dev, cand_idx_dev,                                              \
                                    st_lane, st_ring, user_bound_dev, tile_bound_dev, dense, ph, rows);        \
        break;
    switch (nstep) {
        PK_N_CASE(1)
        PK_N_CASE(2)
        PK_N_CASE(3)
        PK_N_CASE(4)
        PK_N_CASE(5)
        PK_N_CASE(6)
        PK_N_CASE(7)
        PK_N_CASE(8)
        PK_N_CASE(10)
        PK_N_CASE(13)
        PK_N_CASE(16)
    }
#undef PK_N_CASE
    if (rc != PK_OK) return rc;
    PK_CHECK_LAUNCH("score_candidates_kernel");
    return PK_OK;
}

static int pk_score_check_args(const char *who, int64_t n_users, int64_t n_items, int32_t K, const float *Vp_dev,
                               const float *Ep_dev, const int64_t *seen_ptr_dev, const uint64_t *seen_tiles_dev,
                               const int32_t *seen_ntiles_dev, void *state_dev, const float *user_bound_dev,
                               const float *tile_bound_dev, const uint32_t *seen_dense_dev, const int32_t *seen_skip_dev,
                               int32_t dense_tiles, const UserRows *rows = nullptr) {
    PK_REQUIRE(n_users >= 1 && n_items >= 1 && n_items < 0x7fffff00LL, "%s: bad sizes", who);
    if (rows) {
        PK_REQUIRE(rows->E != nullptr && rows->ld >= K && rows->ld % 2 == 0 && ((uintptr_t)rows->E % 16) == 0 && rows->K == K,
                   "%s: E rows must be 16-byte aligned with an even leading dimension >= K", who);
        PK_REQUIRE(rows->extra == nullptr || rows->extra_ld >= 1, "%s: bad stride of the extra term", who);
    }
    PK_REQUIRE(dense_tiles >= 0 && (dense_tiles == 0 || (seen_dense_dev && seen_skip_dev && seen_ptr_dev)),
               "%s: dense seen masks need seen_dense, seen_skip and the seen-tile stream", who);
    PK_REQUIRE(pk_pack_kq(K) > 0, "%s: K=%d unsupported (K <= 256)", who, K);
    PK_REQUIRE(((uintptr_t)Vp_dev % 16) == 0 && ((uintptr_t)Ep_dev % 16) == 0, "%s: alignment", who);
    PK_REQUIRE(state_dev != nullptr && ((uintptr_t)state_dev % 16) == 0, "%s: state buffer", who);
    PK_REQUIRE((seen_ptr_dev == nullptr) == (seen_tiles_dev == nullptr) &&
                   (seen_ptr_dev == nullptr) == (seen_ntiles_dev == nullptr),
               "%s: seen_ptr, seen_tiles, seen_ntiles go together (all or none)", who);
    PK_REQUIRE(rows != nullptr || (user_bound_dev == nullptr) == (tile_bound_dev == nullptr),
               "%s: user_bound and tile_bound go together (both or neither)", who);
    return PK_OK;
}

static int pk_score_candidates_impl(const char *who, void *stream, int64_t n_users, int64_t n_items, int32_t K,
                                    const float *Vp_dev, const float *Ep_dev, const UserRows *rows, const int64_t *seen_ptr_dev,
                                    const uint64_t *seen_tiles_dev, const int32_t *seen_ntiles_dev, int32_t KC, int32_t splits,
                                    float *cand_score_dev, int32_t *cand_idx_dev, void *state_dev, int32_t tiles_per_chunk,
                                    const float *user_bound_dev, const float *tile_bound_dev, const uint32_t *seen_dense_dev,
                                    const int32_t *seen_skip_dev, int32_t dense_tiles) {
    const int rc = pk_score_check_args(who, n_users, n_items, K, Vp_dev, Ep_dev, seen_ptr_dev, seen_tiles_dev, seen_ntiles_dev,
                                       state_dev, user_bound_dev, tile_bound_dev, seen_dense_dev, seen_skip_dev, dense_tiles, rows);
    if (rc != PK_OK) return rc;
    PK_REQUIRE(splits >= 1 && splits * KC <= 64, "%s: need 1 <= splits and splits*KC <= 64", who);
    SeenDense dense{seen_dense_dev, seen_skip_dev, seen_ptr_dev ? dense_tiles : 0};
    return pk_sweep_launches(pk_stream(stream), n_users, n_items, (int)pk_ceil_div(n_items, 32), K, Vp_dev, Ep_dev,
                             seen_ptr_dev, seen_tiles_dev, seen_ntiles_dev, KC, splits, splits, cand_score_dev, cand_idx_dev,
                             state_dev, tiles_per_chunk, user_bound_dev, tile_bound_dev, dense, SweepPhase{0, 0, nullptr, 0},
                             rows ? *rows : UserRows{nullptr, 0, 0, nullptr, 0, 0.0});
}

extern "C" int pk_score_candidates_f32(void *stream, int64_t n_users, int64_t n_items, int32_t K,
                                       const float *Vp_dev, const float *Ep_dev, const int64_t *seen_ptr_dev,
                                       const uint64_t *seen_tiles_dev, const int32_t *seen_ntiles_dev,
                                       int32_t KC, int32_t splits,
                                       float *cand_score_dev, int32_t *cand_idx_dev, void *state_dev,
                                       int32_t tiles_per_chunk, const float *user_bound_dev,
                                       const float *tile_bound_dev, const uint32_t *seen_dense_dev,
                                       const int32_t *seen_skip_dev, int32_t dense_tiles) {
    return pk_score_candidates_impl("pk_score_candidates_f32", stream, n_users, n_items, K, Vp_dev, Ep_dev, nullptr, seen_ptr_dev,
                                    seen_tiles_dev, seen_ntiles_dev, KC, splits, cand_score_dev, cand_idx_dev, state_dev,
                                    tiles_per_chunk, user_bound_dev, tile_bound_dev, seen_dense_dev, seen_skip_dev, dense_tiles);
}

extern "C" int pk_sweep_takes_rows(void) { return 1; }

extern "C" int pk_score_candidates_rows_f32(void *stream, int64_t n_users, int64_t n_items, int32_t K, const float *Vp_dev,
                                            const double *E_dev, int64_t lde, const double *extra_dev, int64_t extra_ld,
                                            double extra_scale, const int64_t *seen_ptr_dev, const uint64_t *seen_tiles_dev,
                                            const int32_t *seen_ntiles_dev, int32_t KC, int32_t splits, float *cand_score_dev,
                                            int32_t *cand_idx_dev, void *state_dev, int32_t tiles_per_chunk,
                                            const float *tile_bound_dev, const uint32_t *seen_dense_dev,
                                            const int32_t *seen_skip_dev, int32_t dense_tiles) {
    const UserRows rows{E_dev, lde, K, extra_dev, extra_ld, extra_scale};
    return pk_score_candidates_impl("pk_score_candidates_rows_f32", stream, n_users, n_items, K, Vp_dev, nullptr, &rows,
                                    seen_ptr_dev, seen_tiles_dev, seen_ntiles_dev, KC, splits, cand_score_dev, cand_idx_dev,
                                    state_dev, tiles_per_chunk, nullptr, tile_bound_dev, seen_dense_dev, seen_skip_dev, dense_tiles);
}

template <int SLOTS>
__global__ __launch_bounds__(256) void merge_candidates_kernel(int64_t n_users, int64_t n_pad, int KC, int lists,
                                                               const float *__restrict__ work_score,
                                                               const int32_t *__restrict__ work_idx,
                                                               float *__restrict__ out_score, int32_t *__restrict__ out_idx) {
    const int lane = threadIdx.x & 63;
    const int64_t user = (int64_t)blockIdx.x * 4 + (threadIdx.x >> 6);
    if (user >= n_pad) return;
    float key[SLOTS];
    int val[SLOTS];
    const int total = lists * KC;
#pragma unroll
    for (int s = 0; s < SLOTS; ++s) {
        const int i = lane + 64 * s;
        key[s] = -INFINITY;
        val[s] = PK_IDX_NONE;
        if (i < total && user < n_users) {
            const int64_t at = ((int64_t)(i / KC) * n_pad + user) * KC + (i % KC);
            const int iv = work_idx[at];
            if (iv >= 0) {
                key[s] = work_score[at];
                val[s] = iv;
            }
        }
    }
    bool extra = false;
#pragma unroll
    for (int s = 0; s < SLOTS; ++s) extra = extra || (lane + 64 * s >= KC && val[s] != PK_IDX_NONE);
    if (!__any(extra)) {
        if (lane < KC) {
            out_score[user * KC + lane] = (user < n_users) ? work_score[user * KC + lane] : -INFINITY;
            out_idx[user * KC + lane] = (user < n_users) ? work_idx[user * KC + lane] : -1;
        }
        return;
    }
    auto before = [](float ka, int va, float kb, int vb) { return ka > kb || (ka == kb && va < vb); };
    constexpr int N = 64 * SLOTS;
    for (int k = 2; k <= N; k <<= 1) {
        for (int j = k >> 1; j > 0; j >>= 1) {
            if (j >= 64) {
                const int ds = j >> 6;
#pragma unroll
                for (int s = 0; s < SLOTS; ++s) {
                    if ((s & ds) == 0 && (s | ds) < SLOTS) {
                        const int i = lane + 64 * s;
                        const bool desc = (i & k) == 0;
                        const int s2 = s | ds;
                        const bool in_order = before(key[s], val[s], key[s2], val[s2]);
                        if (in_order != desc) {
                            const float tk = key[s];
                            const int tv = val[s];
                            key[s] = key[s2];
                            val[s] = val[s2];
                            key[s2] = tk;
                            val[s2] = tv;
                        }
                    }
                }
            } else {
#pragma unroll
                for (int s = 0; s < SLOTS; ++s) {
                    const int i = lane + 64 * s;
                    const float ok = __shfl_xor(key[s], j, 64);
                    const int ov = __shfl_xor(val[s], j, 64);
                    const bool desc = (i & k) == 0;
                    const bool lower = (lane & j) == 0;
                    const bool mine_first = before(key[s], val[s], ok, ov);
                    const bool keep = (mine_first == (lower == desc));
                    if (!keep) {
                        key[s] = ok;
                        val[s] = ov;
                    }
                }
            }
        }
    }
    if (lane < KC) {
        int iv = (val[0] == PK_IDX_NONE) ? -1 : val[0];
        if (lane == KC - 1 && iv < 0 && user < n_users && work_idx[user * KC + KC - 1] == PK_IDX_FLOOR) iv = PK_IDX_FLOOR;
        out_score[user * KC + lane] = key[0];
        out_idx[user * KC + lane] = iv;
    }
}

extern "C" int pk_score_two_phase_plan(int64_t n_users, int64_t n_items, int32_t KC, int32_t *head_tiles, int32_t *splits) {
    PK_REQUIRE(head_tiles && splits, "pk_score_two_phase_plan: null output");
    const int64_t n_tiles = pk_ceil_div(n_items, 32);
    const int64_t groups = pk_ceil_div(n_users, 32);
    int h = (groups <= 1024) ? 32 : 0;
    int s = groups > 768 ? 3 : (groups > 256 ? 7 : 15);
    h = pk_option("score_head_tiles", h);
    s = pk_option("score_phase2_splits", s);
    if (s < 1) s = 1;
    while (s > 1 && (s + 1) * KC > 256) --s;
    if (KC < 1 || KC > 64 || h < 1 || n_tiles < 4 * (int64_t)h) h = 0;
    *head_tiles = h;
    *splits = h ? s : 0;
    return PK_OK;
}

static int pk_score_two_phase_impl(const char *who, void *stream, int64_t n_users, int64_t n_items, int32_t K,
                                   const float *Vp_dev, const float *Ep_dev, const UserRows *rows_in, const int64_t *seen_ptr_dev,
                                   const uint64_t *seen_tiles_dev, const int32_t *seen_ntiles_dev,
                                   int32_t KC, int32_t head_tiles, int32_t splits,
                                   float *work_score_dev, int32_t *work_idx_dev,
                                   float *cand_score_dev, int32_t *cand_idx_dev, void *state_dev,
                                   int32_t tiles_per_chunk, const float *user_bound_dev,
                                   const float *tile_bound_dev, const uint32_t *seen_dense_dev,
                                   const int32_t *seen_skip_dev, int32_t dense_tiles) {
    int rc = pk_score_check_args(who, n_users, n_items, K, Vp_dev, Ep_dev, seen_ptr_dev,
                                 seen_tiles_dev, seen_ntiles_dev, state_dev, user_bound_dev, tile_bound_dev,
                                 seen_dense_dev, seen_skip_dev, dense_tiles, rows_in);
    if (rc != PK_OK) return rc;
    const UserRows rows = rows_in ? *rows_in : UserRows{nullptr, 0, 0, nullptr, 0, 0.0};
    const int n_tiles = (int)pk_ceil_div(n_items, 32);
    PK_REQUIRE((user_bound_dev || rows_in) && tile_bound_dev, "%s: needs the pruning bounds", who);
    PK_REQUIRE(KC >= 1 && KC <= 64 && splits >= 1 && (splits + 1) * KC <= 256 && head_tiles >= 1 && head_tiles < n_tiles,
               "%s: need 1 <= head_tiles < n_tiles and (splits + 1) * KC <= 256", who);
    PK_REQUIRE(work_score_dev && work_idx_dev && cand_score_dev && cand_idx_dev, "%s: null list buffers", who);
    hipStream_t st = pk_stream(stream);
    SeenDense dense{seen_dense_dev, seen_skip_dev, seen_ptr_dev ? dense_tiles : 0};
    const int total_slots = splits + 1;
    rc = pk_sweep_launches(st, n_users, n_items, head_tiles, K, Vp_dev, Ep_dev, seen_ptr_dev, seen_tiles_dev, seen_ntiles_dev,
                           KC, 1, total_slots, work_score_dev, work_idx_dev, state_dev, head_tiles, user_bound_dev,
                           tile_bound_dev, dense, SweepPhase{0, 0, nullptr, 0}, rows);
    if (rc != PK_OK) return rc;
    LaneState *st_lane = static_cast<LaneState *>(state_dev);
    rc = pk_sweep_launches(st, n_users, n_items, n_tiles, K, Vp_dev, Ep_dev, seen_ptr_dev, seen_tiles_dev, seen_ntiles_dev,
                           KC, splits, total_slots, work_score_dev, work_idx_dev, state_dev, tiles_per_chunk, user_bound_dev,
                           tile_bound_dev, dense, SweepPhase{head_tiles, 1, st_lane, 0}, rows);
    if (rc != PK_OK) return rc;
    const int64_t n_pad = pk_ceil_div(n_users, 32) * 32;
    const int slots = (int)pk_ceil_div((int64_t)total_slots * KC, 64);
    dim3 grid((unsigned)pk_ceil_div(n_pad, 4));
#define PK_MERGE(SL)                                                                                               \
    hipLaunchKernelGGL((merge_candidates_kernel<SL>), grid, dim3(256), 0, st, n_users, n_pad, KC, total_slots,     \
                       work_score_dev, work_idx_dev, cand_score_dev, cand_idx_dev)
    if (slots <= 1) PK_MERGE(1);
    else if (slots == 2) PK_MERGE(2);
    else PK_MERGE(4);
#undef PK_MERGE
    PK_CHECK_LAUNCH("merge_candidates_kernel");
    return PK_OK;
}

extern "C" int pk_score_two_phase_f32(void *stream, int64_t n_users, int64_t n_items, int32_t K,
                                      const float *Vp_dev, const float *Ep_dev, const int64_t *seen_ptr_dev,
                                      const uint64_t *seen_tiles_dev, const int32_t *seen_ntiles_dev,
                                      int32_t KC, int32_t head_tiles, int32_t splits,
                                      float *work_score_dev, int32_t *work_idx_dev,
                                      float *cand_score_dev, int32_t *cand_idx_dev, void *state_dev,
                                      int32_t tiles_per_chunk, const float *user_bound_dev,
                                      const float *tile_bound_dev, const uint32_t *seen_dense_dev,
                                      const int32_t *seen_skip_dev, int32_t dense_tiles) {
    return pk_score_two_phase_impl("pk_score_two_phase_f32", stream, n_users, n_items, K, Vp_dev, Ep_dev, nullptr, seen_ptr_dev,
                                   seen_tiles_dev, seen_ntiles_dev, KC, head_tiles, splits, work_score_dev, work_idx_dev,
                                   cand_score_dev, cand_idx_dev, state_dev, tiles_per_chunk, user_bound_dev, tile_bound_dev,
                                   seen_dense_dev, seen_skip_dev, dense_tiles);
}

extern "C" int pk_score_two_phase_rows_f32(void *stream, int64_t n_users, int64_t n_items, int32_t K, const float *Vp_dev,
                                           const double *E_dev, int64_t lde, const double *extra_dev, int64_t extra_ld,
                                           double extra_scale, const int64_t *seen_ptr_dev, const uint64_t *seen_tiles_dev,
                                           const int32_t *seen_ntiles_dev, int32_t KC, int32_t head_tiles, int32_t splits,
                                           float *work_score_dev, int32_t *work_idx_dev, float *cand_score_dev,
                                           int32_t *cand_idx_dev, void *state_dev, int32_t tiles_per_chunk,
                                           const float *tile_bound_dev, const uint32_t *seen_dense_dev,
                                           const int32_t *seen_skip_dev, int32_t dense_tiles) {
    const UserRows rows{E_dev, lde, K, extra_dev, extra_ld, extra_scale};
    return pk_score_two_phase_impl("pk_score_two_phase_rows_f32", stream, n_users, n_items, K, Vp_dev, nullptr, &rows, seen_ptr_dev,
                                   seen_tiles_dev, seen_ntiles_dev, KC, head_tiles, splits, work_score_dev, work_idx_dev,
                                   cand_score_dev, cand_idx_dev, state_dev, tiles_per_chunk, nullptr, tile_bound_dev,
                                   seen_dense_dev, seen_skip_dev, dense_tiles);
}

hipError_t pk_tu_load_score() {
    hipFuncAttributes a;
    return hipFuncGetAttributes(&a, reinterpret_cast<const void *>(&pack_frag_kernel));
}
```

### polara_amd/ops.py

```python
import ctypes as C

import numpy as np
import torch

from . import _lib
from .csr import SPLIT_NNZ


_PTR_KEEP = None


def _ptr(t, offset=0):
    if t is None:
        return None
    if _PTR_KEEP is not None:
        _PTR_KEEP.append(t)
    return C.c_void_p(t.data_ptr() + offset * t.element_size())


def _raw_stream(index):
    return torch._C._cuda_getCurrentRawStream(index)


class _KernelTimer:
# ... 935 lines not shown

    def resid_colnorm2(self, Z, X, theta):
        assert Z.stride(1) == 1 and X.stride(1) == 1 and theta.is_contiguous()
        n, l = Z.shape
        nb = self.lib.pk_resid_blocks(n)
        part = self.empty(nb, l)
        _lib.check(self.lib.pk_resid_colnorm2_f64(self.stream(), n, l, _ptr(Z), Z.stride(0), _ptr(X), X.stride(0),
                                                  _ptr(theta), _ptr(part)), 'pk_resid_colnorm2_f64')
        return part.sum(dim=0)

    def small_mm(self, A, B, transA=False, transB=False):
        A = A.contiguous()
        B = B.contiguous()
        M = A.shape[1] if transA else A.shape[0]
        K = A.shape[0] if transA else A.shape[1]
        N = B.shape[0] if transB else B.shape[1]
        out = self.empty(M, N)
        _lib.check(self.lib.pk_dgemm_small_f64(self.stream(), int(transA), int(transB), M, N, K, _ptr(A),
                                               A.stride(0), _ptr(B), B.stride(0), _ptr(out), out.stride(0)),
                   'pk_dgemm_small_f64')
        return out

    def scale_cols(self, X, s):
        assert X.stride(1) == 1
        _lib.check(self.lib.pk_scale_cols_f64(self.stream(), X.shape[0], X.shape[1], _ptr(X), X.stride(0),
                                              _ptr(s.contiguous())), 'pk_scale_cols_f64')
        return X

    def pack_frag(self, M):
        assert M.stride(1) == 1 and M.dtype == torch.float64
        n, K = M.shape
        out = torch.empty(self.lib.pk_pack_elems(n, K), dtype=torch.float32, device=self.device)
        _lib.check(self.lib.pk_pack_frag_f32(self.stream(), n, K, _ptr(M), M.stride(0), _ptr(out)),
                   'pk_pack_frag_f32')
        return out

    def candidate_capacity(self, topk):
        return self.lib.pk_candidate_capacity(topk)

    def score_splits(self, n_users, KC, prune=False):
        if self.score_splits_override:
            return self.score_splits_override
        if prune and -(-n_users // 32) * 8 > 2048:
            return 1
        return self.lib.pk_score_splits(n_users, KC)

    def pack_frag_bound(self, M, extra=None, extra_scale=0.0):
        assert M.stride(1) == 1 and M.dtype == torch.float64
        n, K = M.shape
        out = torch.empty(self.lib.pk_pack_elems(n, K), dtype=torch.float32, device=self.device)
        bound = torch.empty(n, dtype=torch.float32, device=self.device)
        e_ld = 0 if extra is None else (extra.stride(0) if extra.numel() > 1 else 1)
        with self._timed('pack_frag_bound', (n, K)):
            _lib.check(self.lib.pk_pack_frag_bound_f32(self.stream(), n, K, _ptr(M), M.stride(0), _ptr(out), _ptr(bound),
                                                       _ptr(extra), e_ld, float(extra_scale)), 'pk_pack_frag_bound_f32')
        return out, bound

    def row_norm_bound(self, M):
        assert M.stride(1) == 1
        out = torch.empty(M.shape[0], dtype=torch.float32, device=self.device)
        _lib.check(self.lib.pk_row_norm_bound_f32(self.stream(), M.shape[0], M.shape[1], _ptr(M), M.stride(0),
                                                  _ptr(out)), 'pk_row_norm_bound_f32')
        return out

    def v32_image(self, V, bound, ld):
        assert V.stride(1) == 1 and V.dtype == torch.float64 and bound.dtype == torch.float32
        n, K = int(V.shape[0]), int(V.shape[1])
        out = torch.empty((n, int(ld)), dtype=torch.float32, device=self.device)
        stat = torch.empty(2, dtype=torch.int32, device=self.device)
        _lib.check(self.lib.pk_v32_image_f32(self.stream(), n, K, int(ld), _ptr(V), V.stride(0), _ptr(bound), _ptr(out), _ptr(stat)),
                   'pk_v32_image_f32')
        h = stat.cpu().numpy().view(np.uint32)
        return out, float(np.array([h[0]], dtype=np.uint32).view(np.float32)[0]), not bool(h[1])

    def tile_norm_bound(self, V):
        assert V.stride(1) == 1
        n = V.shape[0]
        work = torch.empty(n, dtype=torch.float32, device=self.device)
        out = torch.empty(-(-n // 32), dtype=torch.float32, device=self.device)
        _lib.check(self.lib.pk_tile_norm_bound_f32(self.stream(), n, V.shape[1], _ptr(V), V.stride(0), _ptr(work),
                                                   _ptr(out)), 'pk_tile_norm_bound_f32')
        return out

    def seen_tiles(self, seen_ptr, seen_idx, n_users, rows_sorted=True):
        tiles = torch.empty(max(int(seen_idx.numel()), 1), dtype=torch.int64, device=self.device)
        ntiles = torch.empty(n_users, dtype=torch.int32, device=self.device)
        max_row = 0
        if not rows_sorted:
            max_row = int((seen_ptr[1:n_users + 1] - seen_ptr[:n_users]).max().item()) if n_users else 0
            if max_row > self.lib.pk_seen_tiles_max_unsorted_row():
                lo, hi = int(seen_ptr[0]), int(seen_ptr[n_users])
                n_cols = int(seen_idx[lo:hi].max().item()) + 1 if hi > lo else 1
                ident = torch.arange(n_cols, dtype=torch.int32, device=self.device)
                ptr0 = (seen_ptr[:n_users + 1] - lo).contiguous()
                idx = seen_idx[lo:hi].contiguous()
                out_i = torch.empty_like(idx)
                dummy = torch.zeros(hi - lo, dtype=torch.float32, device=self.device)
                work = self._work(self.lib.pk_csr_relabel_work_bytes(hi - lo))
                _lib.check(self.lib.pk_csr_relabel_sorted(self.stream(), n_users, n_cols, hi - lo, _ptr(ptr0), _ptr(idx),
                                                          _ptr(dummy), _lib.PK_VAL_F32, _ptr(ident), _ptr(out_i),
                                                          _ptr(torch.empty_like(dummy)), _ptr(work)), 'pk_csr_relabel_sorted')
                seen_idx = torch.cat([seen_idx[:lo], out_i])
                rows_sorted = True
        with self._timed('seen_tiles', (n_users, int(seen_idx.numel()))):
            _lib.check(self.lib.pk_seen_tiles_build(self.stream(), n_users, _ptr(seen_ptr), _ptr(seen_idx),
                                                    1 if rows_sorted else 0, max_row, _ptr(tiles), _ptr(ntiles)),
                       'pk_seen_tiles_build')
        return tiles, ntiles

    def seen_dense(self, seen_ptr, tiles, ntiles, n_users, dense_tiles):
        groups = -(-n_users // 32)
        dense = torch.empty((groups, dense_tiles, 32), dtype=torch.int32, device=self.device)
        skip = torch.empty(n_users, dtype=torch.int32, device=self.device)
        _lib.check(self.lib.pk_seen_dense_build(self.stream(), n_users, _ptr(seen_ptr), _ptr(tiles), _ptr(ntiles), int(dense_tiles),
                                                _ptr(dense), _ptr(skip)), 'pk_seen_dense_build')
        return dense, skip

    def sweep_takes_rows(self, E):
        if not self.lib.pk_sweep_takes_rows():
            return False
        return (E.dtype == torch.float64 and E.dim() == 2 and E.stride(1) == 1 and E.stride(0) % 2 == 0 and E.data_ptr() % 16 == 0)

    @staticmethod
    def _rows_args(E_rows, K):
        E, extra, scale = E_rows
        assert E.shape[1] >= K
        e_ld = 0 if extra is None else extra.stride(0)
        return _ptr(E), E.stride(0), _ptr(extra), int(e_ld), float(scale if extra is not None else 0.0)

    def score_candidates(self, Vp, Ep, n_users, n_items, K, seen_ptr, seen_idx, KC, splits=1, tiles_per_chunk=0,
                         user_bound=None, tile_bound=None, seen_tiles=None, seen_dense=None, E_rows=None):
        n_pad = -(-n_users // 32) * 32
        need = self.lib.pk_score_state_bytes(n_users, splits)
        if self._score_states is None:
            self._score_states = {}
        skey = self.stream_key()
        if skey not in self._score_states or self._score_states[skey].numel() < need:
            self._score_states[skey] = torch.empty(need, dtype=torch.uint8, device=self.device)
        self._score_state = self._score_states[skey]
        cs = torch.empty(splits * n_pad * KC, dtype=torch.float32, device=self.device)
        ci = torch.empty(splits * n_pad * KC, dtype=torch.int32, device=self.device)
        tiles = ntiles = dense = skip = None
        dtiles = 0
        if seen_ptr is not None:
            tiles, ntiles = seen_tiles if seen_tiles is not None else self.seen_tiles(seen_ptr, seen_idx, n_users)
            if seen_dense is not None:
                dense, skip, dtiles = seen_dense
        if E_rows is not None:
            ep, lde, xp, xld, xs = self._rows_args(E_rows, K)
            with self._timed('score_candidates', (n_users, n_items, K)):
                _lib.check(self.lib.pk_score_candidates_rows_f32(self.stream(), n_users, n_items, K, _ptr(Vp), ep, lde, xp, xld, xs,
                                                                 _ptr(seen_ptr), _ptr(tiles), _ptr(ntiles), KC, splits,
                                                                 _ptr(cs), _ptr(ci), _ptr(self._score_state),
                                                                 tiles_per_chunk or self.score_tiles_per_chunk,
                                                                 _ptr(tile_bound), _ptr(dense), _ptr(skip), int(dtiles)),
                           'pk_score_candidates_rows_f32')
            return cs, ci
        with self._timed('score_candidates', (n_users, n_items, K)):
            _lib.check(self.lib.pk_score_candidates_f32(self.stream(), n_users, n_items, K, _ptr(Vp), _ptr(Ep),
                                                        _ptr(seen_ptr), _ptr(tiles), _ptr(ntiles), KC, splits,
                                                        _ptr(cs), _ptr(ci),
                                                        _ptr(self._score_state),
                                                        tiles_per_chunk or self.score_tiles_per_chunk,
                                                        _ptr(user_bound), _ptr(tile_bound), _ptr(dense), _ptr(skip), int(dtiles)),
                       'pk_score_candidates_f32')
        return cs, ci

    def two_phase_plan(self, n_users, n_items, KC):
        h, s = C.c_int32(0), C.c_int32(0)
        _lib.check(self.lib.pk_score_two_phase_plan(int(n_users), int(n_items), int(KC), C.byref(h), C.byref(s)),
                   'pk_score_two_phase_plan')
        return int(h.value), int(s.value)

    def score_two_phase(self, Vp, Ep, n_users, n_items, K, seen_ptr, KC, head_tiles, splits, user_bound, tile_bound,
                        seen_tiles=None, seen_dense=None, tiles_per_chunk=0, E_rows=None):
        n_pad = -(-n_users // 32) * 32
        total = splits + 1
        need = self.lib.pk_score_state_bytes(n_users, total)
        if self._score_states is None:
            self._score_states = {}
        skey = self.stream_key()
        if skey not in self._score_states or self._score_states[skey].numel() < need:
            self._score_states[skey] = torch.empty(need, dtype=torch.uint8, device=self.device)
        self._score_state = self._score_states[skey]
        ws = torch.empty(total * n_pad * KC, dtype=torch.float32, device=self.device)
        wi = torch.empty(total * n_pad * KC, dtype=torch.int32, device=self.device)
        cs = torch.empty(n_pad * KC, dtype=torch.float32, device=self.device)
        ci = torch.empty(n_pad * KC, dtype=torch.int32, device=self.device)
        tiles = ntiles = dense = skip = None
        dtiles = 0
        if seen_ptr is not None:
            tiles, ntiles = seen_tiles
            if seen_dense is not None:
                dense, skip, dtiles = seen_dense
        if E_rows is not None:
            ep, lde, xp, xld, xs = self._rows_args(E_rows, K)
            with self._timed('score_candidates', (n_users, n_items, K)):
                _lib.check(self.lib.pk_score_two_phase_rows_f32(self.stream(), n_users, n_items, K, _ptr(Vp), ep, lde, xp, xld, xs,
                                                                _ptr(seen_ptr), _ptr(tiles), _ptr(ntiles), KC, int(head_tiles),
                                                                int(splits), _ptr(ws), _ptr(wi), _ptr(cs), _ptr(ci),
                                                                _ptr(self._score_state),
                                                                tiles_per_chunk or self.score_tiles_per_chunk,
                                                                _ptr(tile_bound), _ptr(dense), _ptr(skip), int(dtiles)),
                           'pk_score_two_phase_rows_f32')
            return cs, ci
        with self._timed('score_candidates', (n_users, n_items, K)):
            _lib.check(self.lib.pk_score_two_phase_f32(self.stream(), n_users, n_items, K, _ptr(Vp), _ptr(Ep), _ptr(seen_ptr),
                                                       _ptr(tiles), _ptr(ntiles), KC, int(head_tiles), int(splits),
                                                       _ptr(ws), _ptr(wi), _ptr(cs), _ptr(ci), _ptr(self._score_state),
                                                       tiles_per_chunk or self.score_tiles_per_chunk,
                                                       _ptr(user_bound), _ptr(tile_bound), _ptr(dense), _ptr(skip), int(dtiles)),
                       'pk_score_two_phase_f32')
        return cs, ci

    def score_exit_tiles(self, n_users, splits=1):
        groups = -(-n_users // 32)
        rec = self._score_state[:splits * groups * 64 * 16].view(torch.int64).view(splits, groups, 64, 2)
        return rec[:, :, 0, 0].clone()

    def rescore_topk(self, V, E, n_items, seen_ptr, KC, cs, ci, topk, vmax, want_scores=True, splits=1, out=None,
                     rows=None, n_rows_dev=None, e_err=None, e_exact=False, v32=None, flagged=None, item_norm=None,
                     out_perm=None):
        assert V.stride(1) == 1 and E.stride(1) == 1
        assert v32 is None or (v32.dtype == torch.float32 and v32.stride(1) == 1 and v32.shape[1] >= E.shape[1])
        n_users, K = E.shape
        if out is not None:
            out_idx, out_s, flags = out
            assert out_idx.is_contiguous() and flags.is_contiguous() and (out_s is None or out_s.is_contiguous())
        else:
            out_idx = torch.empty(n_users, topk, dtype=torch.int64, device=self.device)
            out_s = self.empty(n_users, topk) if want_scores else None
            flags = torch.empty(n_users, dtype=torch.int32, device=self.device)
        n_rows = n_users if rows is None else int(rows.numel())
        e_ld = 0 if e_err is None else (e_err.stride(0) if e_err.numel() > 1 else 1)
        with self._timed('rescore_topk' if rows is None else 'rescore_topk_refolded', (n_rows, KC, K)):
            fl, fc, fo = flagged if flagged is not None else (None, None, 0)
            assert item_norm is None or (item_norm.dtype == torch.float32 and item_norm.is_contiguous() and item_norm.numel() == n_items)
            args = (self.stream(), n_rows, _ptr(rows), _ptr(n_rows_dev), n_users, n_items, K, _ptr(V),
                    V.stride(0), _ptr(v32), 0 if v32 is None else v32.stride(0), _ptr(E), E.stride(0), _ptr(e_err), e_ld,
                    1 if e_exact else 0, _ptr(seen_ptr), KC, splits, _ptr(cs), _ptr(ci), topk, float(vmax),
                    _ptr(out_idx), _ptr(out_s), _ptr(flags), _ptr(fl), _ptr(fc), int(fo), _ptr(item_norm))
            if out_perm is None:
                _lib.check(self.lib.pk_rescore_topk_rows_norms_f64(*args), 'pk_rescore_topk_rows_norms_f64')
            else:
                assert out_perm.dtype == torch.int64 and out_perm.is_contiguous() and out_perm.numel() == n_users
                _lib.check(self.lib.pk_rescore_topk_rows_perm_f64(*args, _ptr(out_perm)), 'pk_rescore_topk_rows_perm_f64')
        return out_idx, out_s, flags

    def zero_counters(self, n):
        c = torch.empty(int(n), dtype=torch.int32, device=self.device)
        _lib.check(self.lib.pk_zero_i32(self.stream(), _ptr(c), int(n)), 'pk_zero_i32')
        return c

    def flag_compact(self, flags, mask=7):
        n = flags.numel()
        lst = torch.empty(max(n, 1), dtype=torch.int32, device=self.device)
        cnt = torch.empty(1, dtype=torch.int32, device=self.device)
        with self._timed('flag_compact', (n,)):
            _lib.check(self.lib.pk_flag_compact(self.stream(), n, _ptr(flags), int(mask), _ptr(lst), _ptr(cnt)),
                       'pk_flag_compact')
        return lst, cnt

    def fold_rows(self, A, lst, cnt, V, E, row_offset=0):
        assert V.stride(1) == 1 and E.stride(1) == 1 and V.dtype == torch.float64
        with self._timed('fold_rows', (int(lst.numel()),)):
            _lib.check(self.lib.pk_fold_rows_f64(self.stream(), lst.numel(), _ptr(lst), _ptr(cnt), int(row_offset),
                                                 _ptr(A.indptr), _ptr(A.indices), _ptr(A.values), A.val_kind, _ptr(V),
                                                 V.stride(0), V.shape[1], _ptr(E), E.stride(0)), 'pk_fold_rows_f64')

    def score_exact_rows(self, rows, V, E, n_items, seen_ptr, seen_idx, topk):
        n_rows = rows.numel()
        K = E.shape[1]
        out_idx = torch.empty(n_rows, topk, dtype=torch.int64, device=self.device)
        out_s = self.empty(n_rows, topk)
        work = torch.empty(self.lib.pk_exact_work_bytes(n_rows, n_items), dtype=torch.uint8, device=self.device)
        _lib.check(self.lib.pk_score_exact_rows_f64(self.stream(), n_rows, _ptr(rows), n_items, K, _ptr(V),
                                                    V.stride(0), _ptr(E), E.stride(0), _ptr(seen_ptr),
# ... 331 lines not shown
```

### polara_amd/scoring.py

```python
import threading

import numpy as np
import torch

from . import _lib
from .csr import coo_to_csr

EXACT_ROWS_BYTES = 2 << 30
MAX_FUSED_RANK = 256
PACKED_FOLD_IN = True
PACKED_MAX_TOPK = 20
SWEEP_FROM_ROWS = True


class FactorImage:

    def __init__(self, ops, V, fold=None):
        self.ops = ops
        self.V = V.contiguous()
        self.n_items, self.K = self.V.shape
        self.fold = None
        if fold is not None:
            if tuple(fold.shape) != (self.n_items, self.K):
                raise ValueError('fold-in factors of shape %s do not match the item factors %s'
                                 % (tuple(fold.shape), (self.n_items, self.K)))
            self.fold = fold.contiguous()
        self.fold_in = self.V if self.fold is None else self.fold
        self.fused = self.K <= MAX_FUSED_RANK
        self.Vp = ops.pack_frag(self.V) if self.fused else None
        if not self.fused:
            self.vmax = float(torch.linalg.vector_norm(self.V, dim=1).max().item())
            if not np.isfinite(self.vmax) or (self.vmax != 0.0 and not 1e-30 < self.vmax < 1e30):
                raise ValueError('item factors with max row norm %g are outside the range the scoring kernels work in' % self.vmax)
            self.Q20 = self.tile_bound = self.V32x = self.vnorm = None
            self.Kx = self.K
            return
        self.vnorm = ops.row_norm_bound(self.V)
        self.Kx = -(-(self.K + 1) // 4) * 4
        ld = -(-self.Kx // 32) * 32 if self.Kx > 16 else (4 if self.Kx <= 4 else 8 if self.Kx <= 8 else 16)
        if hasattr(ops, 'v32_image'):
            image, self.vmax, finite = ops.v32_image(self.V, self.vnorm, ld)
        else:
            image = torch.zeros(self.n_items, ld, dtype=torch.float32, device=self.V.device)
            image[:, :self.K] = self.V.to(torch.float32)
            image[:, self.K] = self.vnorm
            self.vmax = float(torch.linalg.vector_norm(self.V, dim=1).max().item())
            finite = bool(np.isfinite(self.vmax))
        if not finite or (self.vmax != 0.0 and not 1e-30 < self.vmax < 1e30):
            raise ValueError('item factors with max row norm %g are outside the range the fp32 candidate sweep '
                             'works in (rescale the factors)' % (self.vmax if finite else float('nan')))
        self.Q20 = None
        self.tile_bound = ops.tile_norm_bound(self.V)
        self.V32x = image[:, :self.Kx]
        self.Q20 = ops.q20_encode(self.V) if (PACKED_FOLD_IN and hasattr(ops, 'q20_encode')) else None


def test_csr_from_triplet(test_data, shape, weights=None):
    users, items, fdbk = test_data
    vals = np.asarray(fdbk if weights is None else weights, dtype=np.float64)
    return coo_to_csr(users, items, vals, shape, sum_duplicates=True)


ORDER_USERS_MIN = 8192
HEAD_USERS = 0
_in_pass = threading.local()


def renumbered_test_rows(ops, users):
    ud = ops.to_device(np.ascontiguousarray(users, dtype=np.int64))
    if ud.numel() < 2:
        return torch.zeros_like(ud)
    step = ud[1:] - ud[:-1]
    unsorted, gaps = torch.stack([(step < 0).any(), (step > 1).any() | (ud[0] != 0)]).tolist()
    if unsorted:
        raise AssertionError('the test set must be sorted by users')
    if not gaps:
        return ud
    rows = torch.zeros_like(ud)
    rows[1:] = torch.cumsum((step > 0).to(torch.int64), 0)
    return rows


def _one_batch(n_users, batches, head_users, stats):
    B = int(batches) if batches else -(-n_users // (1 << 22))
    B = max(1, min(B, n_users // 4096)) if n_users >= 4096 else 1
    head = (int(head_users or 0) // 128) * 128
    if stats is not None:
        B, head = 1, 0
    if not (0 < head and 4 * head <= n_users):
        head = 0
    return B, head


def recommend(ops, factors, T, topk, filter_seen=True, return_scores=False, stats=None, prune=True, batches=None,
              approx_fold_in=None, order_users=True, head_users=None, two_phase_ok=True, out=None, queries=None, _out_perm=None):
    lock = getattr(ops, 'pass_lock', None)
    if lock is not None and not getattr(_in_pass, 'held', False):
        with lock:
            _in_pass.held = True
            try:
                return recommend(ops, factors, T, topk, filter_seen, return_scores, stats, prune, batches, approx_fold_in,
                                 order_users, head_users, two_phase_ok, out, queries, _out_perm)
            finally:
                _in_pass.held = False
    n_users, n_items = T.shape
    if out is not None and (return_scores or tuple(out.shape) != (n_users, topk) or out.dtype != torch.int64 or not out.is_contiguous()
                            or not (out.is_cuda or out.is_pinned())):
        raise ValueError('recommend: `out` takes the ids only: a contiguous int64 [n_users x topk] device or pinned host tensor')
    if n_items != factors.n_items:
        raise ValueError('test matrix and item factors disagree on the number of items')
    if topk > n_items:
        raise ValueError('kth(=%d) out of bounds (%d)' % (n_items - topk, n_items))
    if queries is not None and (queries.dim() != 2 or queries.dtype != torch.float64 or queries.stride(1) != 1
                                or tuple(queries.shape) != (n_users, factors.K)):
        raise ValueError('recommend: `queries` must be an fp64 [n_users x K] = [%d x %d] block with unit column stride'
                         % (n_users, factors.K))
    if order_users and prune and factors.fused and n_users >= ORDER_USERS_MIN and hasattr(T, 'by_activity'):
        Tp, perm = T.by_activity()
        if head_users is None:
            head_users = HEAD_USERS
        producer_order = (not return_scores and out is None and getattr(ops, 'lists_in_caller_order', False)
                          and _one_batch(n_users, batches, head_users, stats) == (1, 0)
                          and (ops.candidate_capacity(topk) if factors.fused else 0) > 0)
        res = recommend(ops, factors, Tp, topk, filter_seen, return_scores, stats, prune, batches, approx_fold_in,
                        order_users=False, head_users=head_users, two_phase_ok=two_phase_ok,
                        queries=None if queries is None else queries.index_select(0, perm),
                        _out_perm=perm if producer_order else None)
        if producer_order:
            return res
        if return_scores:
            idx_p, sc_p = res
            out_idx, out_s = torch.empty_like(idx_p), torch.empty_like(sc_p)
            out_idx[perm] = idx_p
            out_s[perm] = sc_p
            return out_idx, out_s
        if out is not None:
            return ops.scatter_rows(res, perm, out=out)
        return ops.scatter_rows(res, perm) if hasattr(ops, 'scatter_rows') else torch.empty_like(res).index_copy_(0, perm, res)
    KC = ops.candidate_capacity(topk) if factors.fused else 0
    K = factors.K
    if KC == 0:
        E = ops.spmm(T, factors.fold_in) if queries is None else queries
        seen_ptr = T.indptr if filter_seen else None
        seen_idx = T.indices if filter_seen else None
        out_idx = torch.empty(n_users, topk, dtype=torch.int64, device=E.device)
        out_s = torch.empty(n_users, topk, dtype=torch.float64, device=E.device)
        per = max(1, int(EXACT_ROWS_BYTES // (n_items * 9 + 16)))
        for s0 in range(0, n_users, per):
            sub = torch.arange(s0, min(n_users, s0 + per), dtype=torch.int32, device=E.device)
            ex_idx, ex_s = ops.score_exact_rows(sub, factors.V, E, n_items, seen_ptr, seen_idx, topk)
            out_idx[s0:s0 + len(sub)] = ex_idx
            out_s[s0:s0 + len(sub)] = ex_s
        if stats is not None:
            stats.update(flagged_users=n_users, candidate_capacity=0, item_splits=0)
        return (out_idx, out_s) if return_scores else out_idx
    if approx_fold_in is None:
        approx_fold_in = not return_scores
    approx_fold_in = (bool(approx_fold_in) and not return_scores and factors.Kx <= 256 and factors.fold is None
                      and queries is None and T.nonneg())
    Kx = factors.Kx if approx_fold_in else K
    Ex = ops.empty(n_users, Kx) if queries is None else queries
    E = Ex[:, :K]
    seen_ptr = T.indptr if filter_seen else None
    seen_idx = T.indices if filter_seen else None
    seen_tiles = T.seen_tiles() if filter_seen else None
    seen_dense = T.seen_dense() if (filter_seen and prune and hasattr(T, 'seen_dense')) else None
    splits = ops.score_splits(n_users, KC, prune)
    use_two_phase = bool(prune and two_phase_ok and hasattr(ops, 'two_phase_plan') and not getattr(ops, 'score_splits_override', 0))
    two_phase = ops.two_phase_plan(n_users, n_items, KC) if use_two_phase else (0, 0)
    out_idx = torch.empty(n_users, topk, dtype=torch.int64, device=E.device)
    out_s = torch.empty(n_users, topk, dtype=torch.float64, device=E.device)
    flags = torch.empty(n_users, dtype=torch.int32, device=E.device)

    refolded = []
    fused_lists = hasattr(ops, 'zero_counters')
    final_list = final_cnt = counters = None
    batch_no = [0]

    def run_batch(u0, u1):
        nb = u1 - u0
        splits = ops.score_splits(nb, KC, prune)
        two_phase = ops.two_phase_plan(nb, n_items, KC) if use_two_phase else (0, 0)
        if approx_fold_in:
            if fold_zeroes:
                pass
            elif factors.Q20 is not None and PACKED_FOLD_IN and topk <= PACKED_MAX_TOPK:
                ops.fold_q20(T, factors.Q20, K, out=Ex, rows=(u0, u1))
            else:
                ops.spmm(T, factors.V32x, out=Ex, rows=(u0, u1))
            w = Ex[u0:u1, K]
        elif queries is not None:
            w = None
        else:
            ops.spmm(T, factors.fold_in, out=Ex, rows=(u0, u1))
            w = None
        Eb = E[u0:u1]
        rows_kw = {}
        if SWEEP_FROM_ROWS and prune and hasattr(ops, 'sweep_takes_rows') and ops.sweep_takes_rows(Eb):
            Ep = ub = None
            rows_kw = {'E_rows': (Eb, w, 1.2e-7)}
        else:
            Ep, ub = ops.pack_frag_bound(Eb, extra=w, extra_scale=1.2e-7)
        if not prune:
            ub = None
        sp = seen_ptr[u0:u1 + 1] if filter_seen else None
        st = (seen_tiles[0], seen_tiles[1][u0:u1]) if seen_tiles is not None else None
        assert u0 % 32 == 0, 'user batches start on a 32-user group boundary (dense seen masks are indexed by group)'
        sd = (seen_dense[0][u0 // 32:], seen_dense[1][u0:u1], seen_dense[2]) if seen_dense is not None else None
        extra = {} if sd is None else {'seen_dense': sd}
        if two_phase[0] and prune:
            cs, ci = ops.score_two_phase(factors.Vp, Ep, nb, n_items, K, sp, KC, two_phase[0], two_phase[1], ub,
                                         factors.tile_bound, seen_tiles=st, seen_dense=sd, **rows_kw)
            splits = 1
        else:
            cs, ci = ops.score_candidates(factors.Vp, Ep, nb, n_items, K, sp, seen_idx, KC, splits,
                                          user_bound=ub, tile_bound=factors.tile_bound if prune else None,
                                          seen_tiles=st, **extra, **rows_kw)
        outs = (out_idx[u0:u1], out_s[u0:u1], flags[u0:u1])
        to_final = (final_list, final_cnt, u0) if fused_lists else None
        if approx_fold_in and fused_lists:
            b = batch_no[0]
            batch_no[0] += 1
            lst, cnt = torch.empty(nb, dtype=torch.int32, device=E.device), counters[1 + b:2 + b]
            first = (lst, cnt, 0)
        else:
            first = to_final
        ops.rescore_topk(factors.V, Eb, n_items, sp, KC, cs, ci, topk, factors.vmax, want_scores=True,
                         splits=splits, out=outs, e_err=w, v32=factors.V32x if approx_fold_in else None, **perm_kw, **(
                             {'flagged': first, 'item_norm': factors.vnorm if approx_fold_in else None} if fused_lists else {}))
        if approx_fold_in:
            if not fused_lists:
                lst, cnt = ops.flag_compact(outs[2], 7)
            if hasattr(ops, 'spmm_flagged') and ops.spmm_flagged_ok(factors.V):
                if hasattr(ops, 'spmm_rows_list'):
                    ops.spmm_rows_list(T, factors.V, Ex, lst, cnt, flags, 7, rows=(u0, u1))
                else:
                    ops.spmm_flagged(T, factors.V, Ex, flags, 7, rows=(u0, u1))
            else:
                ops.fold_rows(T, lst, cnt, factors.V, Ex, row_offset=u0)
            ops.rescore_topk(factors.V, Eb, n_items, sp, KC, cs, ci, topk, factors.vmax, want_scores=True,
                             splits=splits, out=outs, rows=lst, n_rows_dev=cnt, e_err=w, e_exact=True, **perm_kw, **(
                                 {'flagged': to_final} if fused_lists else {}))
            refolded.append(cnt)

    B, head = _one_batch(n_users, batches, head_users, stats)
    one_batch = B == 1 and not head
    perm_kw = {}
    if _out_perm is not None:
        assert one_batch and not return_scores and out is None, 'producer-side order: ids only, one batch'
        perm_kw = {'out_perm': _out_perm}
    fold_zeroes = bool(fused_lists and one_batch and approx_fold_in and factors.Q20 is not None and PACKED_FOLD_IN
                       and topk <= PACKED_MAX_TOPK and hasattr(ops, 'fold_q20_zero'))
    if fused_lists:
        if fold_zeroes:
            counters = ops.fold_q20_zero(T, factors.Q20, K, Ex, 2 + max(B, 2), rows=(0, n_users))
        else:
            counters = ops.zero_counters(2 + max(B, 2))
        final_cnt = counters[0:1]
        final_list = torch.empty(n_users, dtype=torch.int32, device=E.device)
    if one_batch:
        run_batch(0, n_users)
    else:
        if B == 1:
            ranges = [(0, head), (head, n_users)]
        else:
            per = -(-(-(-n_users // B)) // 128) * 128
            ranges = [(u0, min(n_users, u0 + per)) for u0 in range(0, n_users, per)]
        main = torch.cuda.current_stream(E.device)
        side = ops.aux_streams(2)
        for sdev in side:
            sdev.wait_stream(main)
        for b, (u0, u1) in enumerate(ranges):
            with torch.cuda.stream(side[b % 2]):
                run_batch(u0, u1)
        for sdev in side:
            main.wait_stream(sdev)
    lst, cnt = (final_list, final_cnt) if fused_lists else ops.flag_compact(flags, 0x7fffffff)
    ops.score_exact_list(lst, cnt, factors.V, E, n_items, seen_ptr, seen_idx, topk, out_idx, out_s, **perm_kw)
    if stats is not None:
        stats['flagged_users'] = int(cnt.item())
        stats['refolded_users'] = int(sum(int(c.item()) for c in refolded))
        stats['approx_fold_in'] = bool(approx_fold_in)
        stats['candidate_capacity'] = KC
# ... 205 lines not shown
```

Baseline: 190.8 million.

## Add tighter two-term suffix bound for pruning tiles in the candidate sweep

Precomputes per-tile suffix records holding the min/max of the first two item-factor coordinates and the max norm of the remaining coordinates. The row-based sweep kernels build per-user lead terms and a residual norm, and every second step check a tighter bound (exact lead product plus Cauchy-Schwarz on the rest) alongside the existing norm-product bound. The goal is to close more tiles earlier and skip scoring work. In exchange it adds extra registers, per-step record loads and a factor-build kernel, and speed depends on how much tighter the bound is for the data.

After: 190.3 million. About the same (-0.3%).

```diff
diff --git a/include/polara_hip.h b/include/polara_hip.h
--- a/include/polara_hip.h
+++ b/include/polara_hip.h
@@ -179,6 +179,26 @@
                            float *bound_dev, const double *extra_dev, int64_t extra_ld, double extra_scale);
 int pk_tile_norm_bound_f32(void *stream, int64_t n_items, int32_t K, const double *V_dev, int64_t ld,
                            float *work_dev, float *out_dev);
+int32_t pk_sweep_bound_lead(void);
+int pk_tile_bound_records_f32(void *stream, int64_t n_items, int32_t K, const double *V_dev, int64_t ld, float *out_dev);
+int pk_score_candidates_rows_bound_f32(void *stream, int64_t n_users, int64_t n_items, int32_t K, const float *Vp_dev,
+                                       const double *E_dev, int64_t lde, const double *extra_dev, int64_t extra_ld,
+                                       double extra_scale, const int64_t *seen_ptr_dev, const uint64_t *seen_tiles_dev,
+                                       const int32_t *seen_ntiles_dev, int32_t KC, int32_t splits, float *cand_score_dev,
+                                       int32_t *cand_idx_dev, void *state_dev, int32_t tiles_per_chunk,
+                                       const float *tile_bound_dev, const uint32_t *seen_dense_dev,
+                                       const int32_t *seen_skip_dev, int32_t dense_tiles, const float *bound_rec_dev);
+int pk_score_two_phase_rows_bound_f32(void *stream, int64_t n_users, int64_t n_items, int32_t K, const float *Vp_dev,
+                                      const double *E_dev, int64_t lde, const double *extra_dev, int64_t extra_ld,
+                                      double extra_scale, const int64_t *seen_ptr_dev, const uint64_t *seen_tiles_dev,
+                                      const int32_t *seen_ntiles_dev, int32_t KC, int32_t head_tiles, int32_t splits,
+                                      float *work_score_dev, int32_t *work_idx_dev, float *cand_score_dev, int32_t *cand_idx_dev,
+                                      void *state_dev, int32_t tiles_per_chunk, const float *tile_bound_dev,
+                                      const uint32_t *seen_dense_dev, const int32_t *seen_skip_dev, int32_t dense_tiles,
+                                      const float *bound_rec_dev);
+int pk_sweep_bound_eval_f32(void *stream, int64_t n_users, int64_t n_items, int32_t K, const double *E_dev, int64_t lde,
+                            const double *extra_dev, int64_t extra_ld, double extra_scale, const float *tile_bound_dev,
+                            const float *bound_rec_dev, float *out_dev);
 int pk_rescore_topk_f64(void *stream, int64_t n_users, int64_t n_items, int32_t K,
                         const double *V_dev, int64_t ldv, const double *E_dev, int64_t lde,
                         const int64_t *seen_ptr_dev, int32_t KC, int32_t splits,
diff --git a/polara_amd/_lib.py b/polara_amd/_lib.py
--- a/polara_amd/_lib.py
+++ b/polara_amd/_lib.py
@@ -69,6 +69,13 @@
                                                _vp, _vp, _vp, _i32, _vp, _vp, _vp, _i32]),
     'pk_score_two_phase_rows_f32': (C.c_int, [_vp, _i64, _i64, _i32, _vp, _vp, _i64, _vp, _i64, _f64, _vp, _vp, _vp, _i32, _i32, _i32,
                                               _vp, _vp, _vp, _vp, _vp, _i32, _vp, _vp, _vp, _i32]),
+    'pk_sweep_bound_lead': (_i32, []),
+    'pk_tile_bound_records_f32': (C.c_int, [_vp, _i64, _i32, _vp, _i64, _vp]),
+    'pk_score_candidates_rows_bound_f32': (C.c_int, [_vp, _i64, _i64, _i32, _vp, _vp, _i64, _vp, _i64, _f64, _vp, _vp, _vp, _i32, _i32,
+                                                     _vp, _vp, _vp, _i32, _vp, _vp, _vp, _i32, _vp]),
+    'pk_score_two_phase_rows_bound_f32': (C.c_int, [_vp, _i64, _i64, _i32, _vp, _vp, _i64, _vp, _i64, _f64, _vp, _vp, _vp, _i32, _i32, _i32,
+                                                    _vp, _vp, _vp, _vp, _vp, _i32, _vp, _vp, _vp, _i32, _vp]),
+    'pk_sweep_bound_eval_f32': (C.c_int, [_vp, _i64, _i64, _i32, _vp, _i64, _vp, _i64, _f64, _vp, _vp, _vp]),
     'pk_score_two_phase_plan': (C.c_int, [_i64, _i64, _i32, _vp, _vp]),
     'pk_score_two_phase_f32': (C.c_int, [_vp, _i64, _i64, _i32, _vp, _vp, _vp, _vp, _vp, _i32, _i32, _i32, _vp, _vp, _vp, _vp, _vp,
                                          _i32, _vp, _vp, _vp, _vp, _i32]),
diff --git a/polara_amd/csrc/api.cpp b/polara_amd/csrc/api.cpp
--- a/polara_amd/csrc/api.cpp
+++ b/polara_amd/csrc/api.cpp
@@ -15,7 +15,8 @@
 #include <atomic>
 namespace {
 struct Option { const char *name; std::atomic<int> value; std::atomic<bool> set; };
-Option g_options[] = {{"score_boot_tiles", {0}, {false}}, {"score_head_tiles", {0}, {false}}, {"score_phase2_splits", {0}, {false}}};
+Option g_options[] = {{"score_boot_tiles", {0}, {false}}, {"score_head_tiles", {0}, {false}}, {"score_phase2_splits", {0}, {false}},
+                      {"score_tight_bound", {0}, {false}}};
 }
 int pk_option(const char *name, int dflt) {
     for (auto &o : g_options)
diff --git a/polara_amd/csrc/driver.hip b/polara_amd/csrc/driver.hip
--- a/polara_amd/csrc/driver.hip
+++ b/polara_amd/csrc/driver.hip
@@ -1788,7 +1788,7 @@
     Dev inv64;
     DMat V;
     Csr Ts;
-    Dev Vp, tile_bound, V32, tiles, ntiles, dense, skip;
+    Dev Vp, tile_bound, bound_rec, V32, tiles, ntiles, dense, skip;
     Dev vnorm, q20_raw, q20_tab;
     char *q20_img = nullptr;
     int dense_tiles = 0;
@@ -1846,6 +1846,10 @@
         return fail(ctx, PK_E_LAUNCH, "out of device memory (factor images)");
     CK(pk_pack_frag_f32(st, n_items, K, V.p(), K, sv->Vp.as<float>()));
     CK(pk_tile_norm_bound_f32(st, n_items, K, V.p(), K, tb_work.as<float>(), sv->tile_bound.as<float>()));
+    if (K > pk_sweep_bound_lead()) {
+        if (!sv->bound_rec.alloc((size_t)((n_items + 31) / 32) * 8 * 4)) return fail(ctx, PK_E_LAUNCH, "out of device memory (factor images)");
+        CK(pk_tile_bound_records_f32(st, n_items, K, V.p(), K, sv->bound_rec.as<float>()));
+    }
     sv->Kx_full = ((K + 1 + 3) / 4) * 4;
     sv->ld32 = sv->Kx_full > 16 ? ((sv->Kx_full + 31) / 32) * 32 : (sv->Kx_full <= 4 ? 4 : sv->Kx_full <= 8 ? 8 : 16);
     if (sv->Kx_full <= 256 && sv->nonneg) {
@@ -1959,10 +1963,10 @@
         const int32_t *skip_p = (filter_seen && sv->dense_tiles) ? sv->skip.as<int32_t>() : nullptr;
         if (head_tiles) {
             if (from_rows)
-                CK(pk_score_two_phase_rows_f32(st, n_users, n_items, K, sv->Vp.as<float>(), Ex.p(), Kx, w, approx ? Kx : 0, 1.2e-7, seen_ptr,
-                                               tiles, ntiles, KC, head_tiles, splits2, cs.as<float>(), ci.as<int32_t>(), ms.as<float>(),
-                                               mi.as<int32_t>(), state.p, 0, sv->tile_bound.as<float>(), dense_p, skip_p,
-                                               filter_seen ? sv->dense_tiles : 0));
+                CK(pk_score_two_phase_rows_bound_f32(st, n_users, n_items, K, sv->Vp.as<float>(), Ex.p(), Kx, w, approx ? Kx : 0, 1.2e-7,
+                                                     seen_ptr, tiles, ntiles, KC, head_tiles, splits2, cs.as<float>(), ci.as<int32_t>(),
+                                                     ms.as<float>(), mi.as<int32_t>(), state.p, 0, sv->tile_bound.as<float>(), dense_p,
+                                                     skip_p, filter_seen ? sv->dense_tiles : 0, sv->bound_rec.as<float>()));
             else
                 CK(pk_score_two_phase_f32(st, n_users, n_items, K, sv->Vp.as<float>(), Ep.as<float>(), seen_ptr, tiles, ntiles, KC, head_tiles,
                                           splits2, cs.as<float>(), ci.as<int32_t>(), ms.as<float>(), mi.as<int32_t>(), state.p, 0, ub.as<float>(),
@@ -1971,9 +1975,10 @@
             std::swap(ci, mi);
             splits = 1;
         } else if (from_rows) {
-            CK(pk_score_candidates_rows_f32(st, n_users, n_items, K, sv->Vp.as<float>(), Ex.p(), Kx, w, approx ? Kx : 0, 1.2e-7, seen_ptr,
-                                            tiles, ntiles, KC, splits, cs.as<float>(), ci.as<int32_t>(), state.p, 0,
-                                            sv->tile_bound.as<float>(), dense_p, skip_p, filter_seen ? sv->dense_tiles : 0));
+            CK(pk_score_candidates_rows_bound_f32(st, n_users, n_items, K, sv->Vp.as<float>(), Ex.p(), Kx, w, approx ? Kx : 0, 1.2e-7,
+                                                  seen_ptr, tiles, ntiles, KC, splits, cs.as<float>(), ci.as<int32_t>(), state.p, 0,
+                                                  sv->tile_bound.as<float>(), dense_p, skip_p, filter_seen ? sv->dense_tiles : 0,
+                                                  sv->bound_rec.as<float>()));
         } else {
             CK(pk_score_candidates_f32(st, n_users, n_items, K, sv->Vp.as<float>(), Ep.as<float>(), seen_ptr, tiles, ntiles,
                                        KC, splits, cs.as<float>(), ci.as<int32_t>(), state.p, 0, ub.as<float>(), sv->tile_bound.as<float>(),
diff --git a/polara_amd/csrc/score.hip b/polara_amd/csrc/score.hip
--- a/polara_amd/csrc/score.hip
+++ b/polara_amd/csrc/score.hip
@@ -118,6 +118,34 @@
     int64_t extra_ld;
     double extra_scale;
 };
+
+#ifndef PK_BOUND_D
+#define PK_BOUND_D 2
+#endif
+#ifndef PK_BOUND_CADENCE
+#define PK_BOUND_CADENCE 2
+#endif
+struct SweepBound {
+    const float *rec;
+};
+struct BoundUser {
+    float e0, e1, er, cb;
+};
+__device__ __forceinline__ BoundUser pk_bound_user(double e0, double e1, double ss, double ss_rest, double delta) {
+    BoundUser b;
+    b.e0 = (float)e0;
+    b.e1 = (PK_BOUND_D > 1) ? (float)e1 : 0.0f;
+    b.er = (float)(sqrt(ss_rest) * (1.0 + 1e-6) * (1.0 + 1e-7));
+    b.cb = (float)((delta * (PK_BOUND_D + 1) * (1.0 + 1e-6) + 1e-6 * sqrt(ss)) * (1.0 + 1e-7));
+    return b;
+}
+__device__ __forceinline__ float pk_sweep_bound(const BoundUser &b, float en, float tb, float M0, float m0, float M1, float m1,
+                                                float R) {
+    float lead = fmaxf(b.e0 * M0, b.e0 * m0);
+    if (PK_BOUND_D > 1) lead += fmaxf(b.e1 * M1, b.e1 * m1);
+    const float b2 = fmaf(b.er, R, fmaf(b.cb, tb, lead));
+    return fminf(en * tb, b2);
+}
 
 template <int NSTEP, int KC, bool STRIDED, bool DENSE>
 __global__ __launch_bounds__(256) void score_candidates_kernel(
@@ -128,7 +156,8 @@
     float *__restrict__ cand_score, int32_t *__restrict__ cand_idx,
     LaneState *__restrict__ st_lane, uint2 *__restrict__ st_ring,
     const float *__restrict__ user_bound, const float *__restrict__ tile_bound, SeenDense dense,
-    int tile_base, int slot_base, const LaneState *__restrict__ floor_state, int boot_tiles, UserRows rows) {
+    int tile_base, int slot_base, const LaneState *__restrict__ floor_state, int boot_tiles, UserRows rows,
+    SweepBound tight) {
     constexpr int KQ = 2 * NSTEP;
     constexpr bool PAIRED = (KC == 16);
     constexpr int RG = pk_ring_rows(NSTEP, KC);
@@ -164,9 +193,10 @@
 
     float4 e[KQ];
     float en_rows = -1.0f;
+    BoundUser bu{0.0f, 0.0f, 0.0f, 0.0f};
     if (rows.E) {
         double *buf = reinterpret_cast<double *>(&ring[0][0]);
-        double ss = 0.0;
+        double ss = 0.0, ss_rest = 0.0, lead0 = 0.0, lead1 = 0.0;
 #pragma unroll
         for (int s = 0; s < NSTEP; ++s) {
             __builtin_amdgcn_wave_barrier();
@@ -190,17 +220,26 @@
             for (int j = 0; j < 8; ++j) {
                 const double x = mine[j];
                 ss = fma(x, x, ss);
+                if (s == 0 && j < PK_BOUND_D) ss_rest = hi ? fma(x, x, ss_rest) : ss_rest;
+                else ss_rest = fma(x, x, ss_rest);
                 pk_split_bf16((float)x, bh[j], bl[j]);
+            }
+            if (s == 0) {
+                lead0 = buf[ul * 16];
+                lead1 = buf[ul * 16 + 1];
             }
             e[2 * s] = __builtin_bit_cast(float4, make_uint4(bh[0] | (bh[1] << 16), bh[2] | (bh[3] << 16), bh[4] | (bh[5] << 16), bh[6] | (bh[7] << 16)));
             e[2 * s + 1] = __builtin_bit_cast(float4, make_uint4(bl[0] | (bl[1] << 16), bl[2] | (bl[3] << 16), bl[4] | (bl[5] << 16), bl[6] | (bl[7] << 16)));
         }
         __builtin_amdgcn_wave_barrier();
         ss += pk_lane_xor<32>(ss);
+        if (tight.rec) ss_rest += pk_lane_xor<32>(ss_rest);
         if (user < n_users) {
             double b = sqrt(ss) * (1.0 + 1e-6);
-            if (rows.extra) b += rows.extra_scale * rows.extra[user * rows.extra_ld];
+            const double delta = rows.extra ? rows.extra_scale * rows.extra[user * rows.extra_ld] : 0.0;
+            if (rows.extra) b += delta;
             en_rows = (float)(b * (1.0 + 1e-7));
+            if (tight.rec) bu = pk_bound_user(lead0, lead1, ss, ss_rest, delta);
         }
     } else {
 #pragma unroll
@@ -655,10 +694,26 @@
         unsigned m_nxt = 0u;
         if constexpr (DENSE) m_nxt = (tile_begin < dense_tiles) ? dense_row[(int64_t)tile_begin * 32] : 0u;
         float tb = prune ? tile_bound[(tile_begin < n_tiles) ? tile_begin : 0] : 0.0f;
+        const bool tight_on = prune && rows.E != nullptr && tight.rec != nullptr;
+        float4 trec = make_float4(0.0f, 0.0f, 0.0f, 0.0f);
+        float trec_r = 0.0f;
+        if (tight_on) {
+            const int t0 = tile_begin + (PK_BOUND_CADENCE - 1) * S;
+            const float *r = tight.rec + 8 * (int64_t)((t0 < n_tiles) ? t0 : 0);
+            trec = *reinterpret_cast<const float4 *>(r);
+            trec_r = r[4];
+        }
         int step = 0;
         for (int tile = tile_begin; tile < tile_end; tile += S, ++step) {
             if (prune) {
-                const bool open = en * tb > tau;
+                bool open = en * tb > tau;
+                if (tight_on && step % PK_BOUND_CADENCE == PK_BOUND_CADENCE - 1) {
+                    open = pk_sweep_bound(bu, en, tb, trec.x, trec.y, trec.z, trec.w, trec_r) > tau;
+                    const int tn = tile + PK_BOUND_CADENCE * S;
+                    const float *r = tight.rec + 8 * (int64_t)((tn < n_tiles) ? tn : tile);
+                    trec = *reinterpret_cast<const float4 *>(r);
+                    trec_r = r[4];
+                }
                 const unsigned long long ob = __ballot(open);
                 if (ob == 0ull) {
                     pruned = true;
@@ -1087,6 +1142,114 @@
     return PK_OK;
 }
 
+__global__ __launch_bounds__(256) void tile_bound_records_kernel(int64_t n, int K, const double *__restrict__ src, int64_t ld,
+                                                                 float *__restrict__ rec) {
+    const int64_t r = (int64_t)blockIdx.x * blockDim.x + threadIdx.x;
+    float M0 = -INFINITY, m0 = INFINITY, M1 = -INFINITY, m1 = INFINITY, R = 0.0f;
+    if (r < n) {
+        const double *row = src + r * ld;
+        double s = 0.0;
+        for (int k = PK_BOUND_D; k < K; ++k) s = fma(row[k], row[k], s);
+        M0 = __double2float_ru(row[0]);
+        m0 = __double2float_rd(row[0]);
+        if (PK_BOUND_D > 1) {
+            M1 = __double2float_ru(row[1]);
+            m1 = __double2float_rd(row[1]);
+        }
+        R = __double2float_ru(sqrt(s) * (1.0 + 1e-12));
+    }
+#pragma unroll
+    for (int off = 16; off > 0; off >>= 1) {
+        M0 = fmaxf(M0, __shfl_xor(M0, off, 64));
+        m0 = fminf(m0, __shfl_xor(m0, off, 64));
+        M1 = fmaxf(M1, __shfl_xor(M1, off, 64));
+        m1 = fminf(m1, __shfl_xor(m1, off, 64));
+        R = fmaxf(R, __shfl_xor(R, off, 64));
+    }
+    if ((threadIdx.x & 31) == 0 && r < n) {
+        float4 *out = reinterpret_cast<float4 *>(rec + 8 * (r >> 5));
+        out[0] = make_float4(M0, m0, (PK_BOUND_D > 1) ? M1 : 0.0f, (PK_BOUND_D > 1) ? m1 : 0.0f);
+        out[1] = make_float4(R, 0.0f, 0.0f, 0.0f);
+    }
+}
+__global__ __launch_bounds__(64) void tile_bound_suffix_kernel(int64_t n_tiles, float *__restrict__ rec) {
+    const int lane = threadIdx.x;
+    const int64_t seg = (n_tiles + 63) / 64;
+    const int64_t t0 = lane * seg, t1 = (t0 + seg < n_tiles) ? t0 + seg : n_tiles;
+    float run[5] = {-INFINITY, INFINITY, -INFINITY, INFINITY, 0.0f};
+    for (int64_t t = t1 - 1; t >= t0; --t) {
+#pragma unroll
+        for (int c = 0; c < 5; ++c) {
+            const float v = rec[8 * t + c];
+            run[c] = (c == 1 || c == 3) ? fminf(run[c], v) : fmaxf(run[c], v);
+            rec[8 * t + c] = run[c];
+        }
+    }
+    float carry[5] = {-INFINITY, INFINITY, -INFINITY, INFINITY, 0.0f};
+    for (int l = 63; l > 0; --l) {
+#pragma unroll
+        for (int c = 0; c < 5; ++c) {
+            const float v = __shfl(run[c], l);
+            if (lane < l) carry[c] = (c == 1 || c == 3) ? fminf(carry[c], v) : fmaxf(carry[c], v);
+        }
+    }
+    for (int64_t t = t0; t < t1; ++t) {
+#pragma unroll
+        for (int c = 0; c < 5; ++c) {
+            const float v = rec[8 * t + c];
+            rec[8 * t + c] = (c == 1 || c == 3) ? fminf(v, carry[c]) : fmaxf(v, carry[c]);
+        }
+    }
+}
+
+extern "C" int32_t pk_sweep_bound_lead(void) { return PK_BOUND_D; }
+
+extern "C" int pk_tile_bound_records_f32(void *stream, int64_t n_items, int32_t K, const double *V_dev, int64_t ld,
+                                         float *out_dev) {
+    PK_REQUIRE(n_items >= 1 && K > PK_BOUND_D && ld >= K, "pk_tile_bound_records_f32: bad sizes (the rank must exceed %d)", PK_BOUND_D);
+    PK_REQUIRE(out_dev != nullptr && ((uintptr_t)out_dev % 16) == 0, "pk_tile_bound_records_f32: alignment");
+    hipStream_t st = pk_stream(stream);
+    hipLaunchKernelGGL(tile_bound_records_kernel, dim3((unsigned)pk_ceil_div(n_items, 256)), dim3(256), 0, st, n_items, K,
+                       V_dev, ld, out_dev);
+    PK_CHECK_LAUNCH("tile_bound_records_kernel");
+    hipLaunchKernelGGL(tile_bound_suffix_kernel, dim3(1), dim3(64), 0, st, pk_ceil_div(n_items, 32), out_dev);
+    PK_CHECK_LAUNCH("tile_bound_suffix_kernel");
+    return PK_OK;
+}
+
+__global__ __launch_bounds__(64) void sweep_bound_eval_kernel(int64_t n_users, int64_t n_tiles, UserRows rows,
+                                                              const float *__restrict__ tile_bound, SweepBound tight,
+                                                              float *__restrict__ out) {
+    const int64_t u = (int64_t)blockIdx.x * blockDim.x + threadIdx.x;
+    if (u >= n_users) return;
+    const double *row = rows.E + u * rows.ld;
+    double ss = 0.0, ss_rest = 0.0;
+    for (int k = 0; k < rows.K; ++k) {
+        ss = fma(row[k], row[k], ss);
+        if (k >= PK_BOUND_D) ss_rest = fma(row[k], row[k], ss_rest);
+    }
+    const double delta = rows.extra ? rows.extra_scale * rows.extra[u * rows.extra_ld] : 0.0;
+    const float en = (float)((sqrt(ss) * (1.0 + 1e-6) + delta) * (1.0 + 1e-7));
+    const BoundUser bu = pk_bound_user(row[0], (PK_BOUND_D > 1) ? row[1] : 0.0, ss, ss_rest, delta);
+    for (int64_t t = 0; t < n_tiles; ++t) {
+        const float *r = tight.rec + 8 * t;
+        out[u * n_tiles + t] = pk_sweep_bound(bu, en, tile_bound[t], r[0], r[1], r[2], r[3], r[4]);
+    }
+}
+
+extern "C" int pk_sweep_bound_eval_f32(void *stream, int64_t n_users, int64_t n_items, int32_t K, const double *E_dev, int64_t lde,
+                                       const double *extra_dev, int64_t extra_ld, double extra_scale,
+                                       const float *tile_bound_dev, const float *bound_rec_dev, float *out_dev) {
+    PK_REQUIRE(n_users >= 1 && n_items >= 1 && K > PK_BOUND_D && lde >= K, "pk_sweep_bound_eval_f32: bad sizes");
+    PK_REQUIRE(E_dev && tile_bound_dev && bound_rec_dev && out_dev, "pk_sweep_bound_eval_f32: null argument");
+    PK_REQUIRE(extra_dev == nullptr || extra_ld >= 1, "pk_sweep_bound_eval_f32: bad stride of the extra term");
+    const UserRows rows{E_dev, lde, K, extra_dev, extra_ld, extra_scale};
+    hipLaunchKernelGGL(sweep_bound_eval_kernel, dim3((unsigned)pk_ceil_div(n_users, 64)), dim3(64), 0, pk_stream(stream), n_users,
+                       pk_ceil_div(n_items, 32), rows, tile_bound_dev, SweepBound{bound_rec_dev}, out_dev);
+    PK_CHECK_LAUNCH("sweep_bound_eval_kernel");
+    return PK_OK;
+}
+
 extern "C" int32_t pk_candidate_capacity(int32_t topk) {
     if (topk < 1) return 0;
     if (topk <= 10) return 16;
@@ -1110,7 +1273,7 @@
                                const int64_t *seen_ptr, const unsigned long long *seen_tiles,
                                const int32_t *seen_ntiles, float *cs, int32_t *ci,
                                LaneState *st_lane, uint2 *st_ring, const float *user_bound, const float *tile_bound,
-                               SeenDense dense, SweepPhase ph, UserRows rows) {
+                               SeenDense dense, SweepPhase ph, UserRows rows, SweepBound tight) {
     constexpr bool DENSE_OK = (NSTEP <= 8);
     const bool use_dense = dense.tiles > 0 && DENSE_OK && (grid.y == 1 || ph.floor_state != nullptr);
     const SeenDense no_dense{nullptr, nullptr, 0};
@@ -1138,15 +1301,15 @@
     if (grid.y > 1 || ph.floor_state != nullptr)                                                                \
         hipLaunchKernelGGL((score_candidates_kernel<NSTEP, KCV, true, DENSE_OK>), grid, dim3(256), pk_score_lds_bytes(NSTEP, KCV), st, Vp, Ep, n_users, \
                            n_items, n_tiles, split_tiles, chunk_begin, chunk_tiles, seen_ptr, seen_tiles, seen_ntiles, cs, ci, st_lane, st_ring,  \
-                           user_bound, tile_bound, dn, ph.tile_base, ph.slot_base, ph.floor_state, ph.boot_tiles, rows); \
+                           user_bound, tile_bound, dn, ph.tile_base, ph.slot_base, ph.floor_state, ph.boot_tiles, rows, tight); \
     else if (use_dense)                                                                                         \
         hipLaunchKernelGGL((score_candidates_kernel<NSTEP, KCV, false, DENSE_OK>), grid, dim3(256), pk_score_lds_bytes(NSTEP, KCV), st, Vp, Ep, n_users, \
                            n_items, n_tiles, split_tiles, chunk_begin, chunk_tiles, seen_ptr, seen_tiles, seen_ntiles, cs, ci, st_lane, st_ring,  \
-                           user_bound, tile_bound, dn, 0, ph.slot_base, nullptr, ph.boot_tiles, rows);  \
+                           user_bound, tile_bound, dn, 0, ph.slot_base, nullptr, ph.boot_tiles, rows, tight);  \
     else                                                                                                        \
         hipLaunchKernelGGL((score_candidates_kernel<NSTEP, KCV, false, false>), grid, dim3(256), pk_score_lds_bytes(NSTEP, KCV), st, Vp, Ep, n_users, \
                            n_items, n_tiles, split_tiles, chunk_begin, chunk_tiles, seen_ptr, seen_tiles, seen_ntiles, cs, ci, st_lane, st_ring,  \
-                           user_bound, tile_bound, no_dense, 0, ph.slot_base, nullptr, ph.boot_tiles, rows)
+                           user_bound, tile_bound, no_dense, 0, ph.slot_base, nullptr, ph.boot_tiles, rows, tight)
         switch (KC) {
             case 16:
                 PK_LAUNCH(16);
@@ -1204,7 +1367,8 @@
                              const int32_t *seen_ntiles_dev, int32_t KC, int32_t splits, int32_t total_slots,
                              float *cand_score_dev, int32_t *cand_idx_dev, void *state_dev, int32_t tiles_per_chunk,
                              const float *user_bound_dev, const float *tile_bound_dev, SeenDense dense, SweepPhase ph,
-                             UserRows rows = UserRows{nullptr, 0, 0, nullptr, 0, 0.0}) {
+                             UserRows rows = UserRows{nullptr, 0, 0, nullptr, 0, 0.0}, const float *bound_rec_dev = nullptr) {
+    const SweepBound tight{(rows.E && tile_bound_dev && K > PK_BOUND_D && pk_option("score_tight_bound", 1)) ? bound_rec_dev : nullptr};
     const int kq = pk_pack_kq(K);
     const int nstep = pk_nstep(K);
     const int64_t groups = pk_ceil_div(n_users, 32);
@@ -1224,7 +1388,7 @@
                                     split_tiles, tiles_per_chunk, seen_ptr_dev,                                   \
                                     reinterpret_cast<const unsigned long long *>(seen_tiles_dev), seen_ntiles_dev, \
                                     cand_score_dev, cand_idx_dev,                                              \
-                                    st_lane, st_ring, user_bound_dev, tile_bound_dev, dense, ph, rows);        \
+                                    st_lane, st_ring, user_bound_dev, tile_bound_dev, dense, ph, rows, tight); \
         break;
     switch (nstep) {
         PK_N_CASE(1)
@@ -1274,7 +1438,8 @@
                                     const uint64_t *seen_tiles_dev, const int32_t *seen_ntiles_dev, int32_t KC, int32_t splits,
                                     float *cand_score_dev, int32_t *cand_idx_dev, void *state_dev, int32_t tiles_per_chunk,
                                     const float *user_bound_dev, const float *tile_bound_dev, const uint32_t *seen_dense_dev,
-                                    const int32_t *seen_skip_dev, int32_t dense_tiles) {
+                                    const int32_t *seen_skip_dev, int32_t dense_tiles, const float *bound_rec_dev = nullptr) {
+    PK_REQUIRE(((uintptr_t)bound_rec_dev % 16) == 0, "%s: the bound records must be 16-byte aligned", who);
     const int rc = pk_score_check_args(who, n_users, n_items, K, Vp_dev, Ep_dev, seen_ptr_dev, seen_tiles_dev, seen_ntiles_dev,
                                        state_dev, user_bound_dev, tile_bound_dev, seen_dense_dev, seen_skip_dev, dense_tiles, rows);
     if (rc != PK_OK) return rc;
@@ -1283,7 +1448,7 @@
     return pk_sweep_launches(pk_stream(stream), n_users, n_items, (int)pk_ceil_div(n_items, 32), K, Vp_dev, Ep_dev,
                              seen_ptr_dev, seen_tiles_dev, seen_ntiles_dev, KC, splits, splits, cand_score_dev, cand_idx_dev,
                              state_dev, tiles_per_chunk, user_bound_dev, tile_bound_dev, dense, SweepPhase{0, 0, nullptr, 0},
-                             rows ? *rows : UserRows{nullptr, 0, 0, nullptr, 0, 0.0});
+                             rows ? *rows : UserRows{nullptr, 0, 0, nullptr, 0, 0.0}, bound_rec_dev);
 }
 
 extern "C" int pk_score_candidates_f32(void *stream, int64_t n_users, int64_t n_items, int32_t K,
@@ -1312,6 +1477,20 @@
     return pk_score_candidates_impl("pk_score_candidates_rows_f32", stream, n_users, n_items, K, Vp_dev, nullptr, &rows,
                                     seen_ptr_dev, seen_tiles_dev, seen_ntiles_dev, KC, splits, cand_score_dev, cand_idx_dev,
                                     state_dev, tiles_per_chunk, nullptr, tile_bound_dev, seen_dense_dev, seen_skip_dev, dense_tiles);
+}
+
+extern "C" int pk_score_candidates_rows_bound_f32(void *stream, int64_t n_users, int64_t n_items, int32_t K, const float *Vp_dev,
+                                                  const double *E_dev, int64_t lde, const double *extra_dev, int64_t extra_ld,
+                                                  double extra_scale, const int64_t *seen_ptr_dev, const uint64_t *seen_tiles_dev,
+                                                  const int32_t *seen_ntiles_dev, int32_t KC, int32_t splits, float *cand_score_dev,
+                                                  int32_t *cand_idx_dev, void *state_dev, int32_t tiles_per_chunk,
+                                                  const float *tile_bound_dev, const uint32_t *seen_dense_dev,
+                                                  const int32_t *seen_skip_dev, int32_t dense_tiles, const float *bound_rec_dev) {
+    const UserRows rows{E_dev, lde, K, extra_dev, extra_ld, extra_scale};
+    return pk_score_candidates_impl("pk_score_candidates_rows_bound_f32", stream, n_users, n_items, K, Vp_dev, nullptr, &rows,
+                                    seen_ptr_dev, seen_tiles_dev, seen_ntiles_dev, KC, splits, cand_score_dev, cand_idx_dev,
+                                    state_dev, tiles_per_chunk, nullptr, tile_bound_dev, seen_dense_dev, seen_skip_dev, dense_tiles,
+                                    bound_rec_dev);
 }
 
 template <int SLOTS>
@@ -1422,7 +1601,8 @@
                                    float *cand_score_dev, int32_t *cand_idx_dev, void *state_dev,
                                    int32_t tiles_per_chunk, const float *user_bound_dev,
                                    const float *tile_bound_dev, const uint32_t *seen_dense_dev,
-                                   const int32_t *seen_skip_dev, int32_t dense_tiles) {
+                                   const int32_t *seen_skip_dev, int32_t dense_tiles, const float *bound_rec_dev = nullptr) {
+    PK_REQUIRE(((uintptr_t)bound_rec_dev % 16) == 0, "%s: the bound records must be 16-byte aligned", who);
     int rc = pk_score_check_args(who, n_users, n_items, K, Vp_dev, Ep_dev, seen_ptr_dev,
                                  seen_tiles_dev, seen_ntiles_dev, state_dev, user_bound_dev, tile_bound_dev,
                                  seen_dense_dev, seen_skip_dev, dense_tiles, rows_in);
@@ -1438,12 +1618,12 @@
     const int total_slots = splits + 1;
     rc = pk_sweep_launches(st, n_users, n_items, head_tiles, K, Vp_dev, Ep_dev, seen_ptr_dev, seen_tiles_dev, seen_ntiles_dev,
                            KC, 1, total_slots, work_score_dev, work_idx_dev, state_dev, head_tiles, user_bound_dev,
-                           tile_bound_dev, dense, SweepPhase{0, 0, nullptr, 0}, rows);
+                           tile_bound_dev, dense, SweepPhase{0, 0, nullptr, 0}, rows, bound_rec_dev);
     if (rc != PK_OK) return rc;
     LaneState *st_lane = static_cast<LaneState *>(state_dev);
     rc = pk_sweep_launches(st, n_users, n_items, n_tiles, K, Vp_dev, Ep_dev, seen_ptr_dev, seen_tiles_dev, seen_ntiles_dev,
                            KC, splits, total_slots, work_score_dev, work_idx_dev, state_dev, tiles_per_chunk, user_bound_dev,
-                           tile_bound_dev, dense, SweepPhase{head_tiles, 1, st_lane, 0}, rows);
+                           tile_bound_dev, dense, SweepPhase{head_tiles, 1, st_lane, 0}, rows, bound_rec_dev);
     if (rc != PK_OK) return rc;
     const int64_t n_pad = pk_ceil_div(n_users, 32) * 32;
     const int slots = (int)pk_ceil_div((int64_t)total_slots * KC, 64);
@@ -1489,6 +1669,21 @@
                                    seen_dense_dev, seen_skip_dev, dense_tiles);
 }
 
+extern "C" int pk_score_two_phase_rows_bound_f32(void *stream, int64_t n_users, int64_t n_items, int32_t K, const float *Vp_dev,
+                                                 const double *E_dev, int64_t lde, const double *extra_dev, int64_t extra_ld,
+                                                 double extra_scale, const int64_t *seen_ptr_dev, const uint64_t *seen_tiles_dev,
+                                                 const int32_t *seen_ntiles_dev, int32_t KC, int32_t head_tiles, int32_t splits,
+                                                 float *work_score_dev, int32_t *work_idx_dev, float *cand_score_dev,
+                                                 int32_t *cand_idx_dev, void *state_dev, int32_t tiles_per_chunk,
+                                                 const float *tile_bound_dev, const uint32_t *seen_dense_dev,
+                                                 const int32_t *seen_skip_dev, int32_t dense_tiles, const float *bound_rec_dev) {
+    const UserRows rows{E_dev, lde, K, extra_dev, extra_ld, extra_scale};
+    return pk_score_two_phase_impl("pk_score_two_phase_rows_bound_f32", stream, n_users, n_items, K, Vp_dev, nullptr, &rows,
+                                   seen_ptr_dev, seen_tiles_dev, seen_ntiles_dev, KC, head_tiles, splits, work_score_dev,
+                                   work_idx_dev, cand_score_dev, cand_idx_dev, state_dev, tiles_per_chunk, nullptr, tile_bound_dev,
+                                   seen_dense_dev, seen_skip_dev, dense_tiles, bound_rec_dev);
+}
+
 hipError_t pk_tu_load_score() {
     hipFuncAttributes a;
     return hipFuncGetAttributes(&a, reinterpret_cast<const void *>(&pack_frag_kernel));
diff --git a/polara_amd/ops.py b/polara_amd/ops.py
--- a/polara_amd/ops.py
+++ b/polara_amd/ops.py
@@ -1041,6 +1041,26 @@
                                                    _ptr(out)), 'pk_tile_norm_bound_f32')
         return out
 
+    def tile_bound_records(self, V):
+        assert V.stride(1) == 1 and V.dtype == torch.float64
+        n, K = int(V.shape[0]), int(V.shape[1])
+        if K <= self.lib.pk_sweep_bound_lead():
+            return None
+        out = torch.empty((-(-n // 32), 8), dtype=torch.float32, device=self.device)
+        _lib.check(self.lib.pk_tile_bound_records_f32(self.stream(), n, K, _ptr(V), V.stride(0), _ptr(out)),
+                   'pk_tile_bound_records_f32')
+        return out
+
+    def sweep_bound_eval(self, E, tile_bound, bound_rec, n_items, extra=None, extra_scale=0.0):
+        assert E.dtype == torch.float64 and E.stride(1) == 1
+        n_users, K = int(E.shape[0]), int(E.shape[1])
+        out = torch.empty((n_users, -(-int(n_items) // 32)), dtype=torch.float32, device=self.device)
+        e_ld = 0 if extra is None else extra.stride(0)
+        _lib.check(self.lib.pk_sweep_bound_eval_f32(self.stream(), n_users, int(n_items), K, _ptr(E), E.stride(0), _ptr(extra), int(e_ld),
+                                                    float(extra_scale if extra is not None else 0.0), _ptr(tile_bound),
+                                                    _ptr(bound_rec), _ptr(out)), 'pk_sweep_bound_eval_f32')
+        return out
+
     def seen_tiles(self, seen_ptr, seen_idx, n_users, rows_sorted=True):
         tiles = torch.empty(max(int(seen_idx.numel()), 1), dtype=torch.int64, device=self.device)
         ntiles = torch.empty(n_users, dtype=torch.int32, device=self.device)
@@ -1088,7 +1108,7 @@
         return _ptr(E), E.stride(0), _ptr(extra), int(e_ld), float(scale if extra is not None else 0.0)
 
     def score_candidates(self, Vp, Ep, n_users, n_items, K, seen_ptr, seen_idx, KC, splits=1, tiles_per_chunk=0,
-                         user_bound=None, tile_bound=None, seen_tiles=None, seen_dense=None, E_rows=None):
+                         user_bound=None, tile_bound=None, seen_tiles=None, seen_dense=None, E_rows=None, bound_rec=None):
         n_pad = -(-n_users // 32) * 32
         need = self.lib.pk_score_state_bytes(n_users, splits)
         if self._score_states is None:
@@ -1105,6 +1125,17 @@
             tiles, ntiles = seen_tiles if seen_tiles is not None else self.seen_tiles(seen_ptr, seen_idx, n_users)
             if seen_dense is not None:
                 dense, skip, dtiles = seen_dense
+        if E_rows is not None and bound_rec is not None and tile_bound is not None:
+            ep, lde, xp, xld, xs = self._rows_args(E_rows, K)
+            with self._timed('score_candidates', (n_users, n_items, K)):
+                _lib.check(self.lib.pk_score_candidates_rows_bound_f32(self.stream(), n_users, n_items, K, _ptr(Vp), ep, lde, xp, xld, xs,
+                                                                       _ptr(seen_ptr), _ptr(tiles), _ptr(ntiles), KC, splits,
+                                                                       _ptr(cs), _ptr(ci), _ptr(self._score_state),
+                                                                       tiles_per_chunk or self.score_tiles_per_chunk,
+                                                                       _ptr(tile_bound), _ptr(dense), _ptr(skip), int(dtiles),
+                                                                       _ptr(bound_rec)),
+                           'pk_score_candidates_rows_bound_f32')
+            return cs, ci
         if E_rows is not None:
             ep, lde, xp, xld, xs = self._rows_args(E_rows, K)
             with self._timed('score_candidates', (n_users, n_items, K)):
@@ -1132,7 +1163,7 @@
         return int(h.value), int(s.value)
 
     def score_two_phase(self, Vp, Ep, n_users, n_items, K, seen_ptr, KC, head_tiles, splits, user_bound, tile_bound,
-                        seen_tiles=None, seen_dense=None, tiles_per_chunk=0, E_rows=None):
+                        seen_tiles=None, seen_dense=None, tiles_per_chunk=0, E_rows=None, bound_rec=None):
         n_pad = -(-n_users // 32) * 32
         total = splits + 1
         need = self.lib.pk_score_state_bytes(n_users, total)
@@ -1152,6 +1183,18 @@
             tiles, ntiles = seen_tiles
             if seen_dense is not None:
                 dense, skip, dtiles = seen_dense
+        if E_rows is not None and bound_rec is not None:
+            ep, lde, xp, xld, xs = self._rows_args(E_rows, K)
+            with self._timed('score_candidates', (n_users, n_items, K)):
+                _lib.check(self.lib.pk_score_two_phase_rows_bound_f32(self.stream(), n_users, n_items, K, _ptr(Vp), ep, lde, xp, xld, xs,
+                                                                      _ptr(seen_ptr), _ptr(tiles), _ptr(ntiles), KC, int(head_tiles),
+                                                                      int(splits), _ptr(ws), _ptr(wi), _ptr(cs), _ptr(ci),
+                                                                      _ptr(self._score_state),
+                                                                      tiles_per_chunk or self.score_tiles_per_chunk,
+                                                                      _ptr(tile_bound), _ptr(dense), _ptr(skip), int(dtiles),
+                                                                      _ptr(bound_rec)),
+                           'pk_score_two_phase_rows_bound_f32')
+            return cs, ci
         if E_rows is not None:
             ep, lde, xp, xld, xs = self._rows_args(E_rows, K)
             with self._timed('score_candidates', (n_users, n_items, K)):
diff --git a/polara_amd/scoring.py b/polara_amd/scoring.py
--- a/polara_amd/scoring.py
+++ b/polara_amd/scoring.py
@@ -32,7 +32,7 @@
             self.vmax = float(torch.linalg.vector_norm(self.V, dim=1).max().item())
             if not np.isfinite(self.vmax) or (self.vmax != 0.0 and not 1e-30 < self.vmax < 1e30):
                 raise ValueError('item factors with max row norm %g are outside the range the scoring kernels work in' % self.vmax)
-            self.Q20 = self.tile_bound = self.V32x = self.vnorm = None
+            self.Q20 = self.tile_bound = self.bound_rec = self.V32x = self.vnorm = None
             self.Kx = self.K
             return
         self.vnorm = ops.row_norm_bound(self.V)
@@ -51,6 +51,7 @@
                              'works in (rescale the factors)' % (self.vmax if finite else float('nan')))
         self.Q20 = None
         self.tile_bound = ops.tile_norm_bound(self.V)
+        self.bound_rec = ops.tile_bound_records(self.V) if hasattr(ops, 'tile_bound_records') else None
         self.V32x = image[:, :self.Kx]
         self.Q20 = ops.q20_encode(self.V) if (PACKED_FOLD_IN and hasattr(ops, 'q20_encode')) else None
 
@@ -199,6 +200,8 @@
         if SWEEP_FROM_ROWS and prune and hasattr(ops, 'sweep_takes_rows') and ops.sweep_takes_rows(Eb):
             Ep = ub = None
             rows_kw = {'E_rows': (Eb, w, 1.2e-7)}
+            if getattr(factors, 'bound_rec', None) is not None:
+                rows_kw['bound_rec'] = factors.bound_rec
         else:
             Ep, ub = ops.pack_frag_bound(Eb, extra=w, extra_scale=1.2e-7)
         if not prune:
diff --git a/polara_amd/sweep_bound_ref.py b/polara_amd/sweep_bound_ref.py
--- /dev/null
+++ b/polara_amd/sweep_bound_ref.py
@@ -0,0 +1,90 @@
+import numpy as np
+
+LEAD = 2
+F32 = np.float32
+
+
+def f32_up(x):
+    x = np.asarray(x, dtype=np.float64)
+    f = x.astype(F32)
+    return np.where(f.astype(np.float64) < x, np.nextafter(f, F32(np.inf)), f).astype(F32)
+
+
+def f32_down(x):
+    return -f32_up(-np.asarray(x, dtype=np.float64))
+
+
+def _suffix(per_tile, fn):
+    return fn.accumulate(per_tile[::-1])[::-1]
+
+
+def tile_truth(V, d=LEAD):
+    V = np.asarray(V, dtype=np.float64)
+    n, K = V.shape
+    n_tiles = -(-n // 32)
+    pad = n_tiles * 32 - n
+
+    def tiles(x, fill, fn):
+        return fn.reduce(np.r_[x, np.full(pad, fill)].reshape(n_tiles, 32), axis=1)
+    out = np.zeros((n_tiles, 5))
+    for j in range(d):
+        out[:, 2 * j] = _suffix(tiles(V[:, j], -np.inf, np.maximum), np.maximum)
+        out[:, 2 * j + 1] = _suffix(tiles(V[:, j], np.inf, np.minimum), np.minimum)
+    out[:, 4] = _suffix(tiles(np.sqrt((V[:, d:] ** 2).sum(1)), 0.0, np.maximum), np.maximum)
+    return out
+
+
+def tile_records(V, d=LEAD):
+    t = tile_truth(V, d)
+    rec = np.zeros((t.shape[0], 8), dtype=F32)
+    for j in range(d):
+        rec[:, 2 * j] = f32_up(t[:, 2 * j])
+        rec[:, 2 * j + 1] = f32_down(t[:, 2 * j + 1])
+    rec[:, 4] = f32_up(t[:, 4] * (1.0 + 1e-12))
+    return rec
+
+
+def tile_norm_bound(V):
+    V = np.asarray(V, dtype=np.float64)
+    n = V.shape[0]
+    n_tiles = -(-n // 32)
+    nb = (np.sqrt((V ** 2).sum(1)) * (1.0 + 1e-6)).astype(F32)
+    per = np.r_[nb, np.zeros(n_tiles * 32 - n, dtype=F32)].reshape(n_tiles, 32).max(1)
+    return _suffix(per, np.maximum)
+
+
+def user_terms(E, delta=None, d=LEAD):
+    E = np.asarray(E, dtype=np.float64)
+    delta = np.zeros(E.shape[0]) if delta is None else np.asarray(delta, dtype=np.float64)
+    ss = (E ** 2).sum(1)
+    ss_rest = (E[:, d:] ** 2).sum(1)
+    en = ((np.sqrt(ss) * (1.0 + 1e-6) + delta) * (1.0 + 1e-7)).astype(F32)
+    e0 = E[:, 0].astype(F32)
+    e1 = E[:, 1].astype(F32) if d > 1 else np.zeros(E.shape[0], dtype=F32)
+    er = (np.sqrt(ss_rest) * (1.0 + 1e-6) * (1.0 + 1e-7)).astype(F32)
+    cb = ((delta * (d + 1) * (1.0 + 1e-6) + 1e-6 * np.sqrt(ss)) * (1.0 + 1e-7)).astype(F32)
+    return en, e0, e1, er, cb
+
+
+def bound(E, tb, rec, delta=None, d=LEAD, two_term=True):
+    en, e0, e1, er, cb = (x[:, None] for x in user_terms(E, delta, d))
+    tb = np.asarray(tb, dtype=F32)[None, :]
+    cs = en * tb
+    if not two_term:
+        return cs
+    rec = np.asarray(rec, dtype=F32)
+    lead = np.maximum(e0 * rec[None, :, 0], e0 * rec[None, :, 1])
+    if d > 1:
+        lead = lead + np.maximum(e1 * rec[None, :, 2], e1 * rec[None, :, 3])
+    b2 = er * rec[None, :, 4] + (cb * tb + lead)
+    return np.minimum(cs, b2).astype(F32)
+
+
+def suffix_best(E, V):
+    E, V = np.asarray(E, dtype=np.float64), np.asarray(V, dtype=np.float64)
+    n = V.shape[0]
+    n_tiles = -(-n // 32)
+    S = E @ V.T
+    S = np.concatenate([S, np.full((E.shape[0], n_tiles * 32 - n), -np.inf)], axis=1)
+    per = S.reshape(E.shape[0], n_tiles, 32).max(2)
+    return np.maximum.accumulate(per[:, ::-1], axis=1)[:, ::-1]
```
